# santurini/vsrlab

Hardware: AMD Instinct MI355X
Metric: LR frames/sec fwd+bwd, BasicVSR 4x 540p 7-frame clip, 1->8 MI355X (higher is better)
Workload: dtype bf16; 1 GPU; BasicVSR(mid=64,res_blocks=30,x4) fwd+Charbonnier+bwd+clip+Adam, 540x960->2160x3840, 7-frame clip, 2 clips per GPU (BASELINE configs[1]); clips_per_gpu=2, frames=7, res_blocks=30, parallelism=single GPU, arena=full, train_flow=False, trunk_chains=True

## Files before the change

### __graft_entry__.py

```python
import os
import subprocess
import sys

ROOT = os.path.dirname(os.path.abspath(__file__))
if ROOT not in sys.path:
    sys.path.insert(0, ROOT)


def build() -> None:
    env = dict(os.environ)
    env.setdefault("HIPCC", "/opt/rocm/bin/hipcc" if os.path.exists("/opt/rocm/bin/hipcc") else "hipcc")
    subprocess.run(["make", "-C", os.path.join(ROOT, "vsrlab_amd", "csrc"), "-j4"], check=True, env=env)
    try:
        import json
        head = subprocess.run(["git", "-C", ROOT, "rev-parse", "--short=12", "HEAD"], capture_output=True, text=True).stdout.strip()
        dirty = bool(subprocess.run(["git", "-C", ROOT, "status", "--porcelain", "--", "vsrlab_amd/csrc", "include"],
                                    capture_output=True, text=True).stdout.strip())
        if head:
            with open(os.path.join(ROOT, "vsrlab_amd", "lib", "BUILD_INFO.json"), "w") as f:
                json.dump({"git_head": head, "git_dirty_csrc": dirty}, f)
    except Exception:
        pass
    import vsrlab_amd
    lib = vsrlab_amd._lib.load()
    assert lib.vsr_abi_version() == 4
    vsrlab_amd._lib.load_spatial_corr()
    vsrlab_amd._lib.load_jpeg()
    vsrlab_amd._lib.load_warp_taps()


def smoke() -> None:
    import torch
    from oracle import basicvsr_oracle as O
    from vsrlab_amd.vsr.models.RealBasicVSR.modules.basicvsr import BasicVSR
    assert torch.cuda.is_available(), "smoke() needs an MI355X"
    dev = torch.device("cuda:0")
    shape = (1, 3, 3, 32, 32)
    sd = O.keyed_state_dict(O.basicvsr_param_shapes(64, 2, 4))
    g = torch.Generator().manual_seed(0)
    lrs = torch.rand(*shape, generator=g)
    hr = torch.rand(1, 3, 3, 128, 128, generator=g)
    cot = torch.rand(1, 3, 3, 128, 128, generator=g) * 2 - 1
    sr_o, _, grads_o = O.fwd_bwd({k: v.double() for k, v in sd.items()}, lrs.double(), hr.double(), cot=cot.double())
    _, _, g32 = O.fwd_bwd(sd, lrs, hr, cot=cot)
    with O.emulate_bf16():
        sr_e, _, gemu = O.fwd_bwd(sd, lrs, hr, cot=cot)
    keys = sorted(grads_o)
    cat = lambda d: torch.cat([d[k].double().flatten() for k in keys])
    rel = lambda a, b: float((a - b).norm() / b.norm())
    for dtype, g_cpu, floor, t_sr in (("fp32", g32, 2e-4, 1e-3), ("bf16", gemu, 1e-3, None)):
        m = BasicVSR(64, 2, 4, False, False)
        m.load_state_dict(sd, strict=True)
        m = m.to(dev)
        m.compute_dtype = dtype
        sr = m(lrs.to(dev))
        torch.mean(sr * cot.to(dev)).backward()
        torch.cuda.synchronize()
        e_sr = float((sr.detach().cpu().double() - sr_o).abs().max() / sr_o.abs().max())
        grads = {k: p.grad.cpu() for k, p in m.named_parameters() if p.grad is not None}
        assert set(grads) == set(keys)
        e_g, e_cpu = rel(cat(grads), cat(grads_o)), rel(cat(g_cpu), cat(grads_o))
        print(f"smoke[{dtype}]: sr rel err {e_sr:.3e}, gradient rel-L2 {e_g:.3e} (CPU evaluation at this precision: {e_cpu:.3e}) over {len(keys)} tensors")
        if t_sr is None:
            t_sr = 1.5 * max(float((sr_e.double() - sr_o).abs().max() / sr_o.abs().max()), 1e-3)
        assert e_sr < t_sr and e_g <= 1.5 * max(e_cpu, floor), (dtype, e_sr, e_g, e_cpu)
    from vsrlab_amd import functional as VF
    assert VF.chain_timeouts() == 0, "a trunk-chain dependency wait timed out"
    from vsrlab_amd.core.metrics import PSNR, SSIM, MetricCollection
    from vsrlab_amd.core.utils import compute_metric
    same = compute_metric(MetricCollection({"PSNR": PSNR(), "SSIM": SSIM()}), hr.to(dev), hr.to(dev))
    assert same == {"PSNR": 80.0, "SSIM": 1.0}, same
    from vsrlab_amd.vsr.models.VRT.vrt import aligned_input
    clip = lrs.to(dev)
    zero = torch.zeros(1, 2, 2, 32, 32, device=dev)
    al = aligned_input(clip, zero, zero)
    assert al.shape == (1, 3, 27, 32, 32) and torch.equal(al[:, :, :3], clip)
    assert torch.equal(al[:, :2, 3:15], clip[:, 1:].repeat(1, 1, 4, 1, 1)) and not al[:, 2, 3:15].any()
    assert torch.equal(al[:, 1:, 15:], clip[:, :2].repeat(1, 1, 4, 1, 1)) and not al[:, 0, 15:].any()
    print("smoke OK")


if __name__ == "__main__":
    build()
    if len(sys.argv) > 1 and sys.argv[1] == "smoke":
        smoke()
```

### vsrlab_amd/_lib.py

```python
import ctypes
import os
from ctypes import c_char_p, c_float, c_int, c_longlong, c_size_t, c_void_p

_HERE = os.path.dirname(os.path.abspath(__file__))
LIB_PATH = os.environ.get("VSRLAB_AMD_LIB") or os.path.join(_HERE, "lib", "libvsrlab_hip.so")

DT_F32 = 0
DT_BF16 = 1


class BasicVSRDesc(ctypes.Structure):
    _fields_ = [("n", c_int), ("t", c_int), ("h", c_int), ("w", c_int), ("mid_channels", c_int),
                ("res_blocks", c_int), ("upscale", c_int), ("dtype", c_int), ("arena_mode", c_int)]


class DiscDesc(ctypes.Structure):
    _fields_ = [("n", c_int), ("h", c_int), ("w", c_int), ("mid_ch", c_int), ("dtype", c_int)]


class PerceptualDesc(ctypes.Structure):
    _fields_ = [("n", c_int), ("h", c_int), ("w", c_int), ("dtype", c_int), ("need_grad", c_int)]


class AttnDesc(ctypes.Structure):
    _fields_ = [(k, c_int) for k in ("B", "N", "heads", "head_dim", "q0", "k0", "o0", "Nq", "Nk", "Cout", "c_off", "nW", "Nm")] + \
               [("scale", c_float), ("dtype", c_int), ("mask_packed", c_int), ("mask_value", c_float)]


class DeformDesc(ctypes.Structure):
    _fields_ = [(k, c_int) for k in ("N", "Cin", "Cout", "H", "W", "deform_groups", "modulated", "flow_guided")] + \
               [("max_residue", c_float), ("dtype", c_int)]


class MetricsDesc(ctypes.Structure):
    _fields_ = [("planes", c_longlong), ("C", c_int), ("H", c_int), ("W", c_int), ("window_size", c_int),
                ("sigma", c_float), ("c1", c_float), ("c2", c_float), ("clamp_x", c_int), ("clamp_lo", c_float), ("clamp_hi", c_float)]


class RaftCorrDesc(ctypes.Structure):
    _fields_ = [(k, c_int) for k in ("N", "D", "H", "W", "levels", "radius", "dtype")]


class SpatialCorrDesc(ctypes.Structure):
    _fields_ = [(k, c_int) for k in ("N", "C", "H", "W", "patch_h", "patch_w", "stride_h", "stride_w", "pad_h", "pad_w", "dil_h", "dil_w",
                                     "dtype")] + [("scale", c_float)]


class JpegDesc(ctypes.Structure):
    _fields_ = [(k, c_int) for k in ("N", "H", "W", "quality", "x_dtype", "y_dtype")] + \
               [("x_stride", c_longlong * 4), ("y_stride", c_longlong * 4)]


class WarpTapsDesc(ctypes.Structure):
    _fields_ = [(k, c_int) for k in ("N", "D", "C", "H", "W", "taps", "border", "dtype")] + [("x_nstride", c_longlong)]


_P = c_void_p
_SIGNATURES = {
    "vsr_abi_version": (c_int, []),
    "vsr_status_string": (c_char_p, [c_int]),
    "vsr_basicvsr_num_params": (c_int, [ctypes.POINTER(BasicVSRDesc)]),
    "vsr_basicvsr_workspace_bytes": (c_size_t, [ctypes.POINTER(BasicVSRDesc), c_int]),
    "vsr_basicvsr_forward": (c_int, [ctypes.POINTER(BasicVSRDesc), _P, c_int, _P, _P, _P, c_size_t, c_int, _P]),
    "vsr_basicvsr_backward": (c_int, [ctypes.POINTER(BasicVSRDesc), _P, _P, c_int, _P, _P, _P, _P, c_size_t, _P]),
    "vsr_basicvsr_get_flows": (c_int, [ctypes.POINTER(BasicVSRDesc), _P, _P, _P, _P]),
    "vsr_basicvsr_narrow_workspace_bytes": (c_size_t, [ctypes.POINTER(BasicVSRDesc), c_int]),
    "vsr_basicvsr_narrow_forward": (c_int, [ctypes.POINTER(BasicVSRDesc), _P, c_int, _P, _P, _P, c_size_t, c_int, _P]),
    "vsr_basicvsr_narrow_backward": (c_int, [ctypes.POINTER(BasicVSRDesc), _P, _P, c_int, _P, _P, _P, _P, c_size_t, _P]),
    "vsr_basicvsr_narrow_get_flows": (c_int, [ctypes.POINTER(BasicVSRDesc), _P, _P, _P, _P]),
    "vsr_spynet_workspace_bytes": (c_size_t, [c_int, c_int, c_int, c_int, c_int]),
    "vsr_spynet_forward": (c_int, [c_int, c_int, c_int, c_int, _P, c_int, _P, _P, _P, _P, c_size_t, c_int, _P]),
    "vsr_spynet_backward": (c_int, [c_int, c_int, c_int, c_int, _P, c_int, _P, _P, c_size_t, _P]),
    "vsr_spynet_forward_ex": (c_int, [c_int, c_int, c_int, c_int, _P, c_int, _P, _P, c_int, _P, _P, c_size_t, c_int, _P]),
    "vsr_spynet_backward_ex": (c_int, [c_int, c_int, c_int, c_int, _P, _P, c_int, _P, c_int, _P, _P, _P, _P, c_size_t, _P]),
    "vsr_cleaner_workspace_bytes": (c_size_t, [c_int, c_int, c_int, c_int, c_int, c_int, c_int]),
    "vsr_cleaner_narrow_workspace_bytes": (c_size_t, [c_int, c_int, c_int, c_int, c_int, c_int, c_int, c_int]),
    "vsr_cleaner_forward": (c_int, [c_int, c_int, c_int, c_int, c_int, c_int, c_int, _P, c_int, _P, _P, _P, c_size_t, c_int, _P]),
    "vsr_cleaner_backward": (c_int, [c_int, c_int, c_int, c_int, c_int, c_int, c_int, _P, c_int, _P, _P, _P, _P, c_size_t, _P]),
    "vsr_flow_warp_fwd": (c_int, [c_int, _P, _P, _P, c_int, c_int, c_int, c_int, _P]),
    "vsr_flow_warp_bwd": (c_int, [c_int, _P, _P, _P, c_int, c_int, c_int, c_int, _P]),
    "vsr_flow_warp_bwd_flow": (c_int, [c_int, _P, _P, _P, _P, c_int, c_int, c_int, c_int, _P]),
    "vsr_flow_warp_fwd_ex": (c_int, [c_int, _P, _P, _P, c_int, c_int, c_int, c_int, c_int, _P]),
    "vsr_flow_warp_bwd_ex": (c_int, [c_int, _P, _P, _P, c_int, c_int, c_int, c_int, c_int, _P]),
    "vsr_flow_warp_bwd_flow_ex": (c_int, [c_int, _P, _P, _P, _P, c_int, c_int, c_int, c_int, c_int, _P]),
    "vsr_planar_to_pm": (c_int, [c_int, _P, _P, c_int, c_int, c_int, c_int, c_int, _P]),
    "vsr_pm_to_planar": (c_int, [c_int, _P, _P, c_int, c_int, c_int, c_int, c_int, _P]),
    "vsr_conv3x3_c64_fwd": (c_int, [c_int, _P, _P, _P, _P, _P, _P, c_int, c_int, c_int, c_int, _P]),
    "vsr_conv3x3_c64_chain_sync_bytes": (c_size_t, [c_int, c_int, c_int, c_int]),
    "vsr_conv3x3_c64_chain_fwd": (c_int, [_P, _P, _P, c_int, c_int, c_int, c_int, _P, _P]),
    "vsr_conv3x3_c64_dgrad": (c_int, [c_int, _P, _P, _P, _P, _P, _P, c_int, c_int, c_int, c_int, _P]),
    "vsr_conv_layer_fwd": (c_int, [c_int, c_int, _P, c_int, _P, _P, _P, c_int, c_int, _P, _P, c_int, _P, c_int, c_float, c_int, c_int, c_int, c_int, _P]),
    "vsr_conv_layer_bwd_scratch_bytes": (c_size_t, [c_int, c_int, c_int, c_int, c_int]),
    "vsr_conv_layer_bwd": (c_int, [c_int, c_int, _P, c_int, _P, _P, c_int, c_int, _P, _P, _P, _P, c_int, c_int, c_float, c_int, _P, _P, _P, _P,
                                   _P, c_size_t, c_int, c_int, c_int, _P]),
    "vsr_conv3x3_c64_wgrad_slab_floats": (c_size_t, []),
    "vsr_conv3x3_c64_wgrad": (c_int, [c_int, _P, _P, _P, _P, _P, c_int, c_int, c_int, _P]),
    "vsr_charbonnier_scratch_floats": (c_size_t, []),
    "vsr_charbonnier_fwd_bwd": (c_int, [_P, _P, _P, _P, _P, c_longlong, c_float, _P]),
    "vsr_optim_scratch_floats": (c_size_t, []),
    "vsr_adam_clip_step": (c_int, [_P, _P, _P, _P, c_longlong, c_float, c_float, c_float, c_float, c_float, c_int, c_float,
                                   c_float, _P, _P, _P]),
    "vsr_grad_norm": (c_int, [_P, c_longlong, c_float, _P, _P, _P]),
    "vsr_resize_bilinear": (c_int, [_P, _P, c_longlong, c_int, c_int, c_int, c_int, _P]),
    "vsr_disc_workspace_bytes": (c_size_t, [ctypes.POINTER(DiscDesc), c_int]),
    "vsr_disc_forward": (c_int, [ctypes.POINTER(DiscDesc), _P, c_int, _P, _P, _P, c_size_t, c_int, _P]),
    "vsr_disc_backward": (c_int, [ctypes.POINTER(DiscDesc), _P, c_int, _P, _P, _P, _P, c_size_t, _P]),
    "vsr_spectral_norm": (c_int, [_P, _P, _P, _P, _P, c_int, c_int, c_int, _P]),
    "vsr_spectral_norm_backward": (c_int, [_P, _P, _P, _P, _P, _P, c_int, c_int, _P, _P]),
    "vsr_bce_with_logits": (c_int, [_P, c_float, _P, _P, c_longlong, _P]),
    "vsr_perceptual_workspace_bytes": (c_size_t, [ctypes.POINTER(PerceptualDesc)]),
    "vsr_perceptual_loss": (c_int, [ctypes.POINTER(PerceptualDesc), _P, c_int, _P, _P, _P, _P, _P, _P, c_size_t, _P]),
    "vsr_window_attention_fwd": (c_int, [ctypes.POINTER(AttnDesc), _P, _P, _P, _P, _P, _P]),
    "vsr_window_attention_bwd": (c_int, [ctypes.POINTER(AttnDesc), _P, _P, _P, _P, _P, _P, _P, _P, _P]),
    "vsr_mask_pack": (c_int, [_P, _P, c_int, c_int, _P]),
    "vsr_rpb_gather": (c_int, [_P, _P, c_int, _P, c_int, c_int, _P]),
    "vsr_rpb_scatter": (c_int, [_P, _P, c_int, _P, c_int, c_int, _P]),
    "vsr_deform_conv_workspace_bytes": (c_size_t, [ctypes.POINTER(DeformDesc), c_int]),
    "vsr_deform_conv_fwd": (c_int, [ctypes.POINTER(DeformDesc), _P, _P, _P, _P, _P, _P, _P, _P, c_size_t, _P]),
    "vsr_deform_conv_bwd": (c_int, [ctypes.POINTER(DeformDesc), _P, _P, _P, _P, _P, _P, _P, _P, _P, _P, _P, _P, _P, c_size_t, _P]),
    "vsr_deform_offset_mask": (c_int, [ctypes.POINTER(DeformDesc), _P, _P, _P, _P, _P]),
    "vsr_metrics_scratch_bytes": (c_size_t, [ctypes.POINTER(MetricsDesc)]),
    "vsr_psnr_ssim": (c_int, [ctypes.POINTER(MetricsDesc), _P, _P, _P, _P, c_size_t, _P]),
    "vsr_raft_corr_workspace_bytes": (c_size_t, [ctypes.POINTER(RaftCorrDesc), c_int]),
    "vsr_raft_corr_pyramid_fwd": (c_int, [ctypes.POINTER(RaftCorrDesc), _P, _P, _P, c_size_t, _P]),
    "vsr_raft_corr_pyramid_bwd": (c_int, [ctypes.POINTER(RaftCorrDesc), _P, c_size_t, _P, _P, _P]),
    "vsr_raft_corr_lookup_fwd": (c_int, [ctypes.POINTER(RaftCorrDesc), _P, c_size_t, _P, _P, _P]),
    "vsr_raft_corr_lookup_bwd": (c_int, [ctypes.POINTER(RaftCorrDesc), _P, c_size_t, _P, _P, _P, c_size_t, _P]),
}
EXPORTS = tuple(_SIGNATURES)

OTHER_DEBUG_EXPORTS = ("vsr_debug_chain_inject_error", "vsr_debug_chain_item", "vsr_debug_chain_timeouts", "vsr_debug_chain_timing_begin",
                       "vsr_debug_chain_timing_read", "vsr_debug_warp_bwd_gather", "vsr_debug_warp_bwd_gather_c")
_LL = c_longlong
DEBUG_SIGNATURES = {
    "vsr_debug_tail_last2_fwd": (c_int, [c_int, _P, _P, _P, _P, _P, _P, _LL, _P, _P, _LL, c_int, c_int, c_int, c_int, c_int, c_int, c_int, _P]),
    "vsr_debug_tail_last2_dgrad": (c_int, [_P, _LL, _P, _P, c_int, _P, c_int, c_float, _P, c_int, c_int, c_int, _P]),
    "vsr_debug_tail_planar_c64": (c_int, [c_int, _P, _LL, c_int, _P, _P, _P, _P, c_int, c_float, _P, c_int, c_int, c_int, c_int, _P]),
    "vsr_debug_tail_last2_wgrad": (c_int, [c_int, _P, _P, _LL, c_int, _P, _P, _P, c_int, c_int, c_int, _P]),
    "vsr_debug_tail_conv_unshuffle": (c_int, [c_int, _P, _P, _P, c_int, _P, _P, c_int, c_int, c_int, _P]),
    "vsr_debug_tail_ps_dgrad": (c_int, [c_int, _P, _P, _P, _P, _P, c_int, c_int, _P, c_int, c_int, c_int, c_int, c_int, _P]),
    "vsr_debug_tail_ps_wgrads": (c_int, [c_int, _P, _P, c_int, _P, _P, _P, c_int, c_int, c_int, _P]),
    "vsr_debug_trunk_conv": (c_int, [c_int, c_int, c_int, c_int, _P, _P, _P, _P, _P, c_int, c_float, _P, _P, c_int, _P, _P, c_int, c_int,
                                     c_int, c_int, c_int, _P]),
    "vsr_debug_trunk_stem": (c_int, [c_int, c_int, c_int, _P, _P, _LL, _P, _P, _P, _P, c_int, c_float, c_int, c_int, c_int, _P]),
    "vsr_debug_trunk_stem_dgrad": (c_int, [c_int, c_int, c_int, _P, _P, _P, _P, _P, _LL, c_int, c_int, c_int, c_int, _P]),
    "vsr_debug_trunk_point": (c_int, [c_int, c_int, c_int, _P, _P, _P, _P, _P, _P, _P, c_int, c_int, c_int, _P]),
    "vsr_debug_trunk_wgrad_cc": (c_int, [c_int, c_int, c_int, _P, _P, c_int, _P, c_int, c_int, _P, c_int, _P, c_int, c_int, c_int, _P]),
    "vsr_debug_trunk_stem_wgrads": (c_int, [c_int, c_int, c_int, _P, _LL, _P, c_int, _P, _P, c_int, _P, _P, c_int, _P, c_int, c_int, c_int, _P]),
    "vsr_debug_trunk_chain": (c_int, [c_int, c_int, _P, _P, _P, c_int, _P, c_int, c_int, c_int, c_int, _P]),
    "vsr_debug_spy_conv": (c_int, [c_int, c_int, _P, _P, _P, _P, _P, c_int, _P, c_int, c_int, c_int, _P]),
    "vsr_debug_spy_dgrad": (c_int, [c_int, c_int, _P, _P, _P, _P, _P, c_int, c_int, c_int, _P]),
    "vsr_debug_spy_wgrad": (c_int, [c_int, c_int, _P, _P, _P, _P, c_int, _P, c_int, c_int, c_int, _P]),
    "vsr_debug_spy_prepare": (c_int, [c_int, _P, _P, _P, _P, c_int, c_int, c_int, c_int, c_int, c_int, c_int, _P]),
    "vsr_debug_spy_prepare_bwd": (c_int, [c_int, _P, _P, _P, _P, _P, _P, c_int, c_int, c_int, c_int, c_int, c_int, _P]),
    "vsr_debug_spy_dres": (c_int, [c_int, _P, _P, _P, c_int, c_int, c_int, _P]),
    "vsr_debug_spy_planar": (c_int, [c_int, _P, _P, _P, _P, _P, _LL, c_int, c_int, c_int, c_int, _P]),
}

SPATIAL_CORR_LIB_PATH = os.path.join(_HERE, "lib", "libvsrlab_spatial_corr.so")
SPATIAL_CORR_SIGNATURES = {
    "vsr_spatial_corr_workspace_bytes": (c_size_t, [ctypes.POINTER(SpatialCorrDesc)]),
    "vsr_spatial_corr_fwd": (c_int, [ctypes.POINTER(SpatialCorrDesc), _P, _P, _P, _P, c_size_t, _P]),
    "vsr_spatial_corr_bwd": (c_int, [ctypes.POINTER(SpatialCorrDesc), _P, _P, _P, _P, _P, _P, c_size_t, _P]),
}
SPATIAL_CORR_EXPORTS = tuple(SPATIAL_CORR_SIGNATURES)

JPEG_LIB_PATH = os.path.join(_HERE, "lib", "libvsrlab_jpeg.so")
JPEG_SIGNATURES = {
    "vsr_jpeg_workspace_bytes": (c_size_t, [ctypes.POINTER(JpegDesc)]),
    "vsr_jpeg_fwd": (c_int, [ctypes.POINTER(JpegDesc), _P, _P, _P, c_size_t, _P]),
}
JPEG_EXPORTS = tuple(JPEG_SIGNATURES)

WARP_TAPS_LIB_PATH = os.path.join(_HERE, "lib", "libvsrlab_warp_taps.so")
WARP_TAPS_SIGNATURES = {
    "vsr_warp_taps_fwd": (c_int, [ctypes.POINTER(WarpTapsDesc), _P, _P, _P, _P]),
    "vsr_warp_taps_bwd": (c_int, [ctypes.POINTER(WarpTapsDesc), _P, _P, _P, _P, _P]),
    "vsr_warp_taps_clip_fwd": (c_int, [ctypes.POINTER(WarpTapsDesc), _P, _P, _P, _P, _P]),
    "vsr_warp_taps_clip_bwd": (c_int, [ctypes.POINTER(WarpTapsDesc), _P, _P, _P, _P, _P, _P]),
}
WARP_TAPS_EXPORTS = tuple(WARP_TAPS_SIGNATURES)

_lib = None
_spatial_corr_lib = None
_jpeg_lib = None
_warp_taps_lib = None


def load_warp_taps():
    global _warp_taps_lib
    if _warp_taps_lib is None:
        if not os.path.exists(WARP_TAPS_LIB_PATH):
            raise RuntimeError(
                f"vsrlab_amd: HIP library not built ({WARP_TAPS_LIB_PATH} missing). Run "
                "`python -c 'import __graft_entry__ as g; g.build()'` or `make -C vsrlab_amd/csrc`.")
        lib = ctypes.CDLL(WARP_TAPS_LIB_PATH)
        for name, (res, args) in WARP_TAPS_SIGNATURES.items():
            fn = getattr(lib, name)
            fn.restype = res
            fn.argtypes = args
        _warp_taps_lib = lib
    return _warp_taps_lib


def load_jpeg():
    global _jpeg_lib
    if _jpeg_lib is None:
        if not os.path.exists(JPEG_LIB_PATH):
            raise RuntimeError(
                f"vsrlab_amd: HIP library not built ({JPEG_LIB_PATH} missing). Run "
                "`python -c 'import __graft_entry__ as g; g.build()'` or `make -C vsrlab_amd/csrc`.")
        lib = ctypes.CDLL(JPEG_LIB_PATH)
        for name, (res, args) in JPEG_SIGNATURES.items():
            fn = getattr(lib, name)
            fn.restype = res
            fn.argtypes = args
        _jpeg_lib = lib
    return _jpeg_lib


def load_spatial_corr():
    global _spatial_corr_lib
    if _spatial_corr_lib is None:
        if not os.path.exists(SPATIAL_CORR_LIB_PATH):
            raise RuntimeError(
                f"vsrlab_amd: HIP library not built ({SPATIAL_CORR_LIB_PATH} missing). Run "
                "`python -c 'import __graft_entry__ as g; g.build()'` or `make -C vsrlab_amd/csrc`.")
        lib = ctypes.CDLL(SPATIAL_CORR_LIB_PATH)
        for name, (res, args) in SPATIAL_CORR_SIGNATURES.items():
            fn = getattr(lib, name)
            fn.restype = res
            fn.argtypes = args
        _spatial_corr_lib = lib
    return _spatial_corr_lib


def load():
    global _lib
    if _lib is None:
        if not os.path.exists(LIB_PATH):
            raise RuntimeError(
                f"vsrlab_amd: HIP library not built ({LIB_PATH} missing). Run "
                "`python -c 'import __graft_entry__ as g; g.build()'` or `make -C vsrlab_amd/csrc`.")
        lib = ctypes.CDLL(LIB_PATH)
        for name, (res, args) in _SIGNATURES.items():
            fn = getattr(lib, name)
            fn.restype = res
            fn.argtypes = args
        for name, (res, args) in DEBUG_SIGNATURES.items():
            fn = getattr(lib, name, None) if os.environ.get("VSRLAB_AMD_LIB") else getattr(lib, name)
            if fn is not None:
                fn.restype = res
                fn.argtypes = args
        _lib = lib
    return _lib


def check(status, what):
    if status != 0:
        msg = load().vsr_status_string(status).decode()
        raise RuntimeError(f"vsrlab_amd: {what} failed: {msg} (status {status})")
```

### vsrlab_amd/csrc/common.h

```cpp
#pragma once
#include <hip/hip_runtime.h>
#include <stdint.h>

#define VSR_OK 0
#define VSR_ERR_BADARG (-1)
#define VSR_ERR_UNSUPPORTED (-2)
#define VSR_ERR_HIP (-3)
#define VSR_ERR_WORKSPACE (-4)

#define VSR_F32 0
#define VSR_BF16 1

typedef __bf16 bf16_t;
typedef __attribute__((ext_vector_type(8))) __bf16 bf16x8_t;
typedef __attribute__((ext_vector_type(4))) __bf16 bf16x4_t;
typedef __attribute__((ext_vector_type(4))) short s16x4_t;
typedef __attribute__((ext_vector_type(16))) float f32x16_t;
typedef __attribute__((ext_vector_type(4))) float f32x4_t;

#define VSR_MAX_SRC 4
#define VSR_MAX_Z 4

enum { ACT_NONE = 0, ACT_RELU = 1, ACT_LEAKY = 2 };
enum { MASK_NONE = 0, MASK_RELU = 1, MASK_LEAKY = 2, MASK_RELU_BITS = 3, MASK_LEAKY_BITS = 4 };
enum { EPI_NHWC = 0, EPI_PLANAR = 1 };

struct ConvArgs {
    const void* src[VSR_MAX_SRC];
    long long src_nstride[VSR_MAX_SRC];
    int src_oy[VSR_MAX_SRC], src_ox[VSR_MAX_SRC];
    int in_step, Hs, Ws;
    int N, H, W;
    const void* wpack;
    long long w_zstride;
    const float* bias;
    int bias_zstride;
    int nz;
    void* dst[VSR_MAX_Z];
    long long dst_nstride;
    int out_step, Hd, Wd;
    int out_oy[VSR_MAX_Z], out_ox[VSR_MAX_Z];
    int CD;
    int cout_real;
    int act;
    const void* res[VSR_MAX_Z];
    const void* aux[VSR_MAX_Z];
    int mask_mode;
    const float* pres;
    const float* base_lr;
    long long base_nstride;
    int base_h, base_w, base_scale;
    void* sign_out[VSR_MAX_Z];
    const void* sign_bits[VSR_MAX_Z];
    float leaky_slope;
    int planar_c;
    int unshuffle;
    long long unshuffle_plane;
};
static inline __host__ __device__ float vsr_slope(float s) { return s != 0.f ? s : 0.1f; }

#define VSR_WG_MAXSEG 8
struct WgradArgs {
    const void* x[VSR_WG_MAXSEG];
    const void* dy[VSR_WG_MAXSEG];
    long long x_nstride, dy_nstride;
    int nseg;
    int N, H, W;
    int x_step, x_oy, x_ox, Hx, Wx;
    int dy_step, dy_oy, dy_ox, Hy, Wy;
    float* slab;
    int tap_begin;
    int x_ctotal, x_coff;
    int dy_ctotal, dy_coff;
    int dy_planar_c;
    int slab_stride;
    int ntiles_x, ntiles_y;
    int pair_ksplit, pair_nsl, pair_ncob, pair_views;
};

static inline __host__ __device__ int cdiv(int a, int b) { return (a + b - 1) / b; }
static inline int grid_for(long long total, int block = 256) {
    long long g = (total + block - 1) / block;
    return (int)(g < 1 ? 1 : (g > 256 * 16 ? 256 * 16 : g));
}

static inline __host__ __device__ int pm_ws(int W) { return (W + 31) >> 5; }
static inline __host__ __device__ long long pm_image_elems(int H, int W, int C) { return (long long)H * pm_ws(W) * 32 * C; }
static inline __host__ __device__ long long pm_off(int y, int x, int chunk, int W, int C) {
    const int seg = x >> 5;
    return (((long long)y * pm_ws(W) + seg) * (C >> 3) + chunk) * 256 + (x & 31) * 8;
}

static inline __host__ __device__ int pm_acc_chan(int mb, int row) { return 8 * (4 * (mb >> 1) + (row >> 2)) + 4 * (mb & 1) + (row & 3); }
#define PM_LANE_PIXEL(l15) (((l15) >= 4 && (l15) < 12) ? 2 * ((l15) - 4) : ((l15) < 4 ? 2 * (l15) + 1 : 2 * ((l15) - 8) + 1))

struct TileWalk { int first, end, stride; };
static inline __device__ TileWalk xcd_tile_walk(int total, int block, int nblocks) {
    TileWalk w;
    if (nblocks >= 8 && (nblocks & 7) == 0) {
        const int xcd = block & 7, j = block >> 3;
        const int lo = (int)((long long)xcd * total / 8), hi = (int)((long long)(xcd + 1) * total / 8);
        w.first = lo + j; w.end = hi; w.stride = nblocks >> 3;
    } else {
        w.first = block; w.end = total; w.stride = nblocks;
    }
    return w;
}

#define VSR_MAX_DEVICES 32
struct VsrDevOnce { bool done[VSR_MAX_DEVICES] = {}; };
static inline int vsr_set_max_dynamic_lds(VsrDevOnce& once, const void* kernel, int bytes) {
    int dev = 0;
    if (hipGetDevice(&dev) != hipSuccess) return VSR_ERR_HIP;
    if (dev < 0 || dev >= VSR_MAX_DEVICES) return VSR_ERR_UNSUPPORTED;
    if (!__atomic_load_n(&once.done[dev], __ATOMIC_ACQUIRE)) {
        if (hipFuncSetAttribute(kernel, hipFuncAttributeMaxDynamicSharedMemorySize, bytes) != hipSuccess) return VSR_ERR_HIP;
        __atomic_store_n(&once.done[dev], true, __ATOMIC_RELEASE);
    }
    return VSR_OK;
}

static inline int vsr_num_cus() {
    static int cus[VSR_MAX_DEVICES] = {};
    int dev = 0;
    if (hipGetDevice(&dev) != hipSuccess || dev < 0 || dev >= VSR_MAX_DEVICES) return 256;
    int v = __atomic_load_n(&cus[dev], __ATOMIC_RELAXED);
    if (v == 0) {
        hipDeviceProp_t prop;
        v = (hipGetDeviceProperties(&prop, dev) == hipSuccess && prop.multiProcessorCount > 0) ? prop.multiProcessorCount : 256;
        __atomic_store_n(&cus[dev], v, __ATOMIC_RELAXED);
    }
    return v;
}

#include <cstdlib>
struct VsrEnvSwitches {
    bool generic_conv, generic_wgrad, single_stream;
    int wide2_max_wg;
};
static inline const VsrEnvSwitches& vsr_env() {
    static const VsrEnvSwitches s = [] {
        auto on = [](const char* n) { const char* e = getenv(n); return e && e[0] == '1'; };
        VsrEnvSwitches v;
        v.generic_conv = on("VSRLAB_AMD_GENERIC_CONV");
        v.generic_wgrad = on("VSRLAB_AMD_GENERIC_WGRAD");
        v.single_stream = on("VSRLAB_AMD_SINGLE_STREAM");
        const char* e = getenv("VSRLAB_AMD_WIDE2_MAX_WG");
        v.wide2_max_wg = e ? atoi(e) : 0;
        return v;
    }();
    return s;
}

#define HIP_CHECK_RET(expr)                                   \
    do {                                                      \
        hipError_t _e = (expr);                               \
        if (_e != hipSuccess) return VSR_ERR_HIP;             \
    } while (0)
```

### vsrlab_amd/csrc/engine.hip

```cpp
#include <vector>
#include "recipes.h"
#include "spynet_engine.h"

namespace {

struct Plan {
    VsrBasicVSRDesc d = {};
    int C = 64, CO = 64;
    bool sb = false;
    bool bwd = false, flowgrad = false;
    bool diet = false;
    int rb = 0, n = 0, t = 0, h = 0, w = 0, dtype = VSR_F32;
    int scale = 4, ups = 2;
    bool unsh = false;
    size_t es = 4;
    size_t px1 = 0;
    size_t s_elems = 0;
    size_t stem_w[2] = {}, stem_wd[2] = {}, stem_b[2] = {};
    std::vector<size_t> blk_w[2], blk_wd[2], blk_b[2];
    size_t point_w = 0, point_wd = 0, point_b = 0;
    size_t up_w[2] = {}, up_wd[2] = {}, up_b[2] = {};
    size_t last0_w = 0, last0_wd = 0, last0_b = 0, last2_w = 0, last2_wd = 0, last2_b = 0;
    SpyPlan spy;
    size_t flows = 0;
    std::vector<size_t> Wp[2], X[2], A[2];
    std::vector<size_t> SB[2];
    std::vector<size_t> feat[2];
    size_t scratchA[2] = {}, scratchW[2] = {};
    std::vector<size_t> Pt, U0, U1, C0;
    std::vector<size_t> SBC0;
    std::vector<size_t> SBPt;
    std::vector<size_t> SBX0[2];
    std::vector<size_t> G0[2], G1[2], DX[2];
    std::vector<size_t> dFeatB, dFF;
    size_t S[2] = {}, dWp[2] = {}, slab[2] = {};
    size_t far_cnt = 0;
    size_t chain_sync[2] = {0, 0};
    bool chains = true;
    size_t G_C0 = 0, G_U1 = 0, G_U0 = 0, G_P = 0;
    bool hrdef = false;
    std::vector<size_t> GU1f, GU0f, GPf;
    size_t dflows = 0;
    size_t stem_wd_lr[2] = {};
    size_t total = 0;

    size_t xoff(int dir, int i, int b) const { return X[dir][(size_t)i * (rb + 1) + b]; }
    size_t aoff(int dir, int i, int b) const { return A[dir][(size_t)i * rb + b]; }
    size_t sboff(int dir, int i, int b) const { return SB[dir][(size_t)i * rb + b]; }
    size_t g1off(int dir, int i, int b) const { return diet ? G1[dir][b & 1] : G1[dir][(size_t)i * rb + b]; }
    size_t dxoff(int dir, int i, int b) const { return diet ? DX[dir][b & 1] : DX[dir][(size_t)i * (rb + 1) + b]; }

    int build(const VsrBasicVSRDesc& desc, int mode, bool narrow = false) {
        d = desc; bwd = mode >= 1; flowgrad = mode >= 2;
        { const char* e = getenv("VSRLAB_AMD_CHAIN"); chains = !(e && e[0] == '0'); }
        if (d.arena_mode != 0 && d.arena_mode != 1) return VSR_ERR_BADARG;
        diet = bwd && d.arena_mode == 1;
        rb = d.res_blocks; n = d.n; t = d.t; h = d.h; w = d.w; dtype = d.dtype;
        scale = d.upscale; ups = scale / 2; unsh = false;
        const bool width_ok = narrow ? (d.mid_channels == 16 || d.mid_channels == 32) : d.mid_channels == 64;
        if (!width_ok || (scale != 4 && scale != 2) || rb < 1 || n < 1 || t < 1 || t > 32 || h < 1 || w < 1) return VSR_ERR_UNSUPPORTED;
        if (dtype != VSR_F32 && dtype != VSR_BF16) return VSR_ERR_BADARG;
        const int C = d.mid_channels;
        this->C = C; CO = C < 32 ? 32 : C;
        sb = bwd && dtype == VSR_BF16 && C == 64;
        es = esize(dtype);
        px1 = (size_t)n * pm_image_elems(h, w, C);
        s_elems = (size_t)n * h * w * C;
        const size_t a2 = (size_t)n * pm_image_elems(2 * h, 2 * w, C) * es, a4 = (size_t)n * pm_image_elems(scale * h, scale * w, C) * es;
        const size_t a4h = (size_t)n * pm_image_elems(scale * h, scale * w, 64) * es;
        Bump b;
        const size_t w64 = (size_t)9 * CO * C * es;
        for (int dir = 0; dir < 2; ++dir) {
            stem_w[dir] = b.take(w64 + (size_t)9 * CO * 16 * es);
            stem_wd[dir] = b.take(w64);
            stem_b[dir] = b.take(C * 4);
            blk_w[dir].resize(2 * rb); blk_wd[dir].resize(2 * rb); blk_b[dir].resize(2 * rb);
            for (int k = 0; k < 2 * rb; ++k) { blk_w[dir][k] = b.take(w64); blk_wd[dir][k] = b.take(w64); blk_b[dir][k] = b.take(C * 4); }
        }
        point_w = b.take((size_t)2 * CO * C * es); point_wd = b.take((size_t)2 * CO * C * es); point_b = b.take(C * 4);
        for (int k = 0; k < 2; ++k) { up_w[k] = b.take(4 * w64); up_wd[k] = b.take(4 * w64); up_b[k] = b.take(4 * C * 4); }
        last0_w = b.take((size_t)9 * 64 * C * es); last0_wd = b.take((size_t)9 * CO * 64 * es); last0_b = b.take(64 * 4);
        last2_w = b.take((size_t)9 * 32 * 64 * es); last2_wd = b.take((size_t)9 * 64 * 16 * es); last2_b = b.take(64 * 4);
        if (t > 1) spy.plan(b, 2 * n * (t - 1), n * t, h, w, dtype);
        flows = b.take((size_t)2 * n * (t > 1 ? t - 1 : 1) * 2 * h * w * 4);
        const size_t a1 = px1 * es;
        for (int dir = 0; dir < 2; ++dir) {
            Wp[dir].assign(t, 0); feat[dir].assign(t, 0);
            if (bwd) {
                X[dir].assign((size_t)t * (rb + 1), 0); A[dir].assign((size_t)t * rb, 0); SB[dir].assign((size_t)t * rb, 0);
                SBX0[dir].assign(t, 0);
                const size_t sbytes = sb ? (size_t)n * cdiv(h, 8) * cdiv(w, 32) * 2048 : 256;
                for (int i = 0; i < t; ++i) {
                    SBX0[dir][i] = b.take(sbytes);
                    Wp[dir][i] = b.take(a1);
                    for (int k = 0; k <= rb; ++k) X[dir][(size_t)i * (rb + 1) + k] = b.take(a1);
                    for (int k = 0; k < rb; ++k) A[dir][(size_t)i * rb + k] = b.take(a1);
                    for (int k = 0; k < rb; ++k) SB[dir][(size_t)i * rb + k] = b.take(sbytes);
                    feat[dir][i] = xoff(dir, i, rb);
                }
            } else {
                for (int i = 0; i < t; ++i) feat[dir][i] = b.take(a1);
            }
        }
        for (int dir = 0; dir < 2; ++dir) { scratchA[dir] = b.take(a1); scratchW[dir] = b.take(a1); }
        const int nrec = bwd ? t : 1;
        Pt.assign(t, 0); U0.assign(t, 0); U1.assign(t, 0); C0.assign(t, 0);
        for (int i = 0; i < nrec; ++i) {
            Pt[i] = b.take(a1);
            if (diet && i > 0) { U0[i] = U0[0]; U1[i] = U1[0]; C0[i] = C0[0]; } else { U0[i] = b.take(a2); U1[i] = ups == 2 ? b.take(a4) : U0[i]; C0[i] = b.take(a4h); }
        }
        for (int i = nrec; i < t; ++i) { Pt[i] = Pt[0]; U0[i] = U0[0]; U1[i] = U1[0]; C0[i] = C0[0]; }
        SBC0.assign(t, 0); SBPt.assign(t, 0);
        if (sb)
            for (int i = 0; i < t; ++i) {
                SBC0[i] = b.take((size_t)n * cdiv(scale * h, 8) * cdiv(scale * w, 32) * 2048);
                SBPt[i] = b.take((size_t)n * cdiv(h, 8) * cdiv(w, 32) * 2048);
            }
        if (bwd) {
            for (int dir = 0; dir < 2; ++dir) {
                G0[dir].assign(t, 0);
                for (int i = 0; i < t; ++i) G0[dir][i] = b.take(a1);
                if (diet) {
                    G1[dir].assign(2, 0); DX[dir].assign(2, 0);
                    for (int k = 0; k < 2; ++k) { G1[dir][k] = b.take(a1); DX[dir][k] = b.take(a1); }
                } else if (dir == 0) {
                    G1[dir].assign((size_t)t * rb, 0); DX[dir].assign((size_t)t * (rb + 1), 0);
                    for (int i = 0; i < t; ++i) {
                        for (int k = 0; k < rb; ++k) G1[dir][(size_t)i * rb + k] = b.take(a1);
                        for (int k = 1; k <= rb; ++k) DX[dir][(size_t)i * (rb + 1) + k] = b.take(a1);
                    }
                } else {
                    G1[dir] = G1[0]; DX[dir] = DX[0];
                }
            }
            dFeatB.assign(t, 0); dFF.assign(t, 0);
            for (int i = 0; i < t; ++i) { dFeatB[i] = b.take(a1); dFF[i] = b.take(a1); }
            for (int dir = 0; dir < 2; ++dir) { S[dir] = b.take(s_elems * 8); dWp[dir] = b.take(a1); }
            far_cnt = b.take((size_t)2 * 32 * 4);
            G_C0 = b.take(a4h); G_P = b.take(a1);
            unsh = !diet && dtype == VSR_BF16 && !vsr_env().generic_conv && C == 64;
            const size_t gu1 = unsh && 4 * a2 > a4 ? 4 * a2 : a4, gu0 = unsh && 4 * a1 > a2 ? 4 * a1 : a2;
            if (ups == 2) { if (diet) { G_U1 = C0[0]; G_U0 = U1[0]; } else { G_U1 = b.take(gu1); G_U0 = b.take(gu0); } }
            else { G_U0 = diet ? C0[0] : b.take(gu0); G_U1 = G_U0; }
            hrdef = unsh;
            GU1f.assign(t, G_U1); GU0f.assign(t, G_U0); GPf.assign(t, G_P);
            if (hrdef)
                for (int i = 1; i < t; ++i) {
                    GU0f[i] = b.take(gu0);
                    GU1f[i] = ups == 2 ? b.take(gu1) : GU0f[i];
                    GPf[i] = b.take(a1);
                }
            for (int k = 0; k < 2; ++k) slab[k] = b.take(wgrad_slab_bytes());
        }
        for (int dir = 0; dir < 2; ++dir) chain_sync[dir] = sb ? b.take(vsr_chain_sync_bytes(VSR_CHAIN_MAX_LAYERS, n, h, w)) : 0;
        dflows = 0;
        if (flowgrad && t > 1) {
            dflows = b.take((size_t)2 * n * (t - 1) * 2 * h * w * 4);
            spy.plan_save(b, dtype);
        }
        if (flowgrad) {
            for (int dir = 0; dir < 2; ++dir) stem_wd_lr[dir] = b.take((size_t)9 * 32 * C * es);
        }
        total = b.off;
        return VSR_OK;
    }
};

Ctx engine_ctx(const Plan& p, char* ws, hipStream_t st, int lane) {
    return Ctx(ws, st, p.dtype, p.C, p.bwd ? reinterpret_cast<float*>(ws + p.slab[lane]) : nullptr);
}

struct PIdx {
    int rb;
    int ups = 2;
    int trunk_base(int dir) const { return dir * (2 + 4 * rb); }
    int stem_w(int dir) const { return trunk_base(dir); }
    int stem_b(int dir) const { return trunk_base(dir) + 1; }
    int blk_w(int dir, int k) const { return trunk_base(dir) + 2 + 2 * k; }
    int blk_b(int dir, int k) const { return trunk_base(dir) + 3 + 2 * k; }
    int point_w() const { return 2 * (2 + 4 * rb); }
    int point_b() const { return point_w() + 1; }
    int up_w(int k) const { return point_w() + 2 + 2 * k; }
    int up_b(int k) const { return up_w(k) + 1; }
    int last0_w() const { return point_w() + 2 + 2 * ups; }
    int last0_b() const { return last0_w() + 1; }
    int last2_w() const { return last0_w() + 2; }
    int last2_b() const { return last0_w() + 3; }
    int spy_base() const { return last0_w() + 4; }
    int spy_w(int lvl, int j) const { return spy_base() + (lvl * NSPY + j) * 2; }
    int spy_b(int lvl, int j) const { return spy_w(lvl, j) + 1; }
    int spy_mean() const { return spy_base() + 60; }
    int spy_std() const { return spy_base() + 61; }
    int count() const { return spy_base() + 62; }
};

int pack_all_collect(const Ctx& c, const Plan& p, const float* const* prm);
int pack_all(const Ctx& c, const Plan& p, const float* const* prm) {
    std::vector<VsrPackDesc> descs;
    descs.reserve(512);
    c.batch = &descs;
    const int rc = pack_all_collect(c, p, prm);
    c.batch = nullptr;
    if (rc != VSR_OK) return rc;
    return vsr_launch_pack_multi(descs.data(), (int)descs.size(), c.st);
}

int pack_all_collect(const Ctx& c, const Plan& p, const float* const* prm) {
    const PIdx ix{p.rb, p.ups};
    const int C = p.C, CO = p.CO;
    for (int dir = 0; dir < 2; ++dir) {
        const float* sw = prm[ix.stem_w(dir)];
        CK(c.pack_stem(sw, c.at(p.stem_w[dir]), true));
        CK(c.pack_bias(prm[ix.stem_b(dir)], c.at(p.stem_b[dir]), C));
        if (p.bwd) CK(c.pack_stem_dgrad(sw, c.at(p.stem_wd[dir])));
        if (p.flowgrad) CK(c.pack_stem_dlr(sw, c.at(p.stem_wd_lr[dir]), true));
        for (int k = 0; k < 2 * p.rb; ++k) {
            CK(c.pack_cc(3, prm[ix.blk_w(dir, k)], c.at(p.blk_w[dir][k]), 0));
            if (p.bwd) CK(c.pack_cc(3, prm[ix.blk_w(dir, k)], c.at(p.blk_wd[dir][k]), 1));
            CK(c.pack_bias(prm[ix.blk_b(dir, k)], c.at(p.blk_b[dir][k]), C));
        }
    }
    CK(c.pack_point(prm[ix.point_w()], c.at(p.point_w), 0));
    if (p.bwd) CK(c.pack_point(prm[ix.point_w()], c.at(p.point_wd), 1));
    CK(c.pack_bias(prm[ix.point_b()], c.at(p.point_b), C));
    for (int k = 0; k < p.ups; ++k) {
        CK(c.pack_ps(prm[ix.up_w(k)], c.at(p.up_w[k]), 0));
        if (p.bwd) CK(c.pack_ps(prm[ix.up_w(k)], c.at(p.up_wd[k]), 1));
        CK(c.pack_ps_bias(prm[ix.up_b(k)], (float*)c.at(p.up_b[k])));
    }
    CK(c.pack(prm[ix.last0_w()], c.at(p.last0_w), 9, 64, C, 64, C, C, 0, 1, 0, 0));
    if (p.bwd) CK(c.pack(prm[ix.last0_w()], c.at(p.last0_wd), 9, CO, 64, C, 64, C, 0, 1, 0, 1));
    CK(c.pack_bias(prm[ix.last0_b()], c.at(p.last0_b), 64));
    CK(c.pack(prm[ix.last2_w()], c.at(p.last2_w), 9, 32, 64, 3, 64, 64, 0, 1, 0, 0));
    if (p.bwd) CK(c.pack(prm[ix.last2_w()], c.at(p.last2_wd), 9, 64, 16, 64, 3, 64, 0, 1, 0, 1));
    CK(c.pack_bias(prm[ix.last2_b()], c.at(p.last2_b), 3));
    if (p.t > 1) CK(vsr::spynet_pack(c, p.spy, prm, ix.spy_base()));
    return VSR_OK;
}

bool chain_on(const Plan& p) { return p.chains && p.chain_sync[0] && p.chain_sync[1] && 2 * p.rb <= VSR_CHAIN_MAX_LAYERS; }
unsigned chain_off(size_t o) { return (unsigned)(o >> 8); }
int chain_launch(const ChainArgs& a, hipStream_t st) {
    const size_t img_bytes = (size_t)pm_image_elems(a.H, a.W, 64) * 2, sb_bytes = (size_t)cdiv(a.H, 8) * cdiv(a.W, 32) * 2048;
    if (a.N > 1 && img_bytes * 3 * a.N > ((size_t)192 << 20) && cdiv(a.H, 8) * cdiv(a.W, 32) >= 2 * vsr_num_cus()) {
        for (int m = 0; m < a.N; ++m) {
            ChainArgs b = a;
            b.N = 1;
            const unsigned di = (unsigned)((m * img_bytes) >> 8), ds = (unsigned)((m * sb_bytes) >> 8);
            for (int l = 0; l < a.nlayers; ++l) {
                ChainLayer& L = b.layer[l];
                L.src += di; L.dst += di;
                if (L.res != 0xffffffffu) L.res += di;
                if (L.sbits != 0xffffffffu) L.sbits += ds;
                if (L.sout != 0xffffffffu) L.sout += ds;
            }
            CK(chain_launch(b, st));
        }
        return VSR_OK;
    }
    return vsr_launch_conv3x3_chain(a, vsr_num_cus(), st);
}
int trunk_chain_forward(const Ctx& c, const Plan& p, int dir, int i) {
    ChainArgs a = {};
    a.base = c.ws; a.sync = (unsigned*)c.at(p.chain_sync[dir]); a.N = p.n; a.H = p.h; a.W = p.w; a.nlayers = 2 * p.rb;
    for (int b = 0; b < p.rb; ++b) {
        ChainLayer& l1 = a.layer[2 * b];
        l1 = {chain_off(p.xoff(dir, i, b)), chain_off(p.aoff(dir, i, b)), 0xffffffffu, 0xffffffffu, chain_off(p.sboff(dir, i, b)),
              chain_off(p.blk_w[dir][2 * b]), chain_off(p.blk_b[dir][2 * b]), CHAIN_RELU};
        ChainLayer& l2 = a.layer[2 * b + 1];
        l2 = {chain_off(p.aoff(dir, i, b)), chain_off(p.xoff(dir, i, b + 1)), chain_off(p.xoff(dir, i, b)), 0xffffffffu, 0xffffffffu,
              chain_off(p.blk_w[dir][2 * b + 1]), chain_off(p.blk_b[dir][2 * b + 1]), CHAIN_SKIP};
    }
    return chain_launch(a, c.st);
}
int trunk_chain_backward(const Ctx& c, const Plan& p, int dir, int i) {
    ChainArgs a = {};
    a.base = c.ws; a.sync = (unsigned*)c.at(p.chain_sync[dir]); a.N = p.n; a.H = p.h; a.W = p.w;
    int L = 0;
    for (int b = p.rb - 1; b >= 0; --b) {
        a.layer[L++] = {chain_off(p.dxoff(dir, i, b + 1)), chain_off(p.g1off(dir, i, b)), 0xffffffffu, chain_off(p.sboff(dir, i, b)), 0xffffffffu,
                        chain_off(p.blk_wd[dir][2 * b + 1]), 0xffffffffu, CHAIN_MASK};
        if (b > 0)
            a.layer[L++] = {chain_off(p.g1off(dir, i, b)), chain_off(p.dxoff(dir, i, b)), chain_off(p.dxoff(dir, i, b + 1)), 0xffffffffu, 0xffffffffu,
                            chain_off(p.blk_wd[dir][2 * b]), 0xffffffffu, CHAIN_SKIP};
    }
    a.nlayers = L;
    return chain_launch(a, c.st);
}

int trunk_forward(const Ctx& c, const Plan& p, int dir, int i, const void* warped, const float* lrs) {
    const int n = p.n, h = p.h, w = p.w, rb = p.rb;
    void* x = p.bwd ? c.at(p.xoff(dir, i, 0)) : c.at(p.feat[dir][i]);
    {
        CK(c.stem(true, warped, lrs + (size_t)i * 3 * h * w, (long long)p.t * 3 * h * w, c.at(p.stem_w[dir]), c.fat(p.stem_b[dir]), x, ACT_LEAKY, 0.f, n, h, w));
        if (p.sb) CK(vsr_launch_sign_bits_c64(x, c.at(p.SBX0[dir][i]), n, h, w, c.st));
    }
    if (chain_on(p)) return trunk_chain_forward(c, p, dir, i);
    for (int b = 0; b < rb; ++b) {
        void* act = p.bwd ? c.at(p.aoff(dir, i, b)) : c.at(p.scratchA[dir]);
        void* xn = p.bwd ? c.at(p.xoff(dir, i, b + 1)) : x;
        CK(c.conv(3, x, c.at(p.blk_w[dir][2 * b]), c.fat(p.blk_b[dir][2 * b]), act, ACT_RELU, nullptr, nullptr, 0, n, h, w,
                    p.sb ? c.at(p.sboff(dir, i, b)) : nullptr));
        CK(c.conv(3, act, c.at(p.blk_w[dir][2 * b + 1]), c.fat(p.blk_b[dir][2 * b + 1]), xn, ACT_NONE, x, nullptr, 0, n, h, w));
        x = xn;
    }
    return VSR_OK;
}

int last0_forward(const Ctx& c, const Plan& p, int i, void* sign_out) {
    const int S = p.scale;
    if (p.C == 64)
        return c.conv(3, c.at(p.U1[i]), c.at(p.last0_w), c.fat(p.last0_b), c.at(p.C0[i]), ACT_LEAKY, nullptr, nullptr, 0, p.n, S * p.h, S * p.w, sign_out);
    ConvArgs a = conv_args(p.n, S * p.h, S * p.w, c.C);
    a.src[0] = c.at(p.U1[i]); a.wpack = c.at(p.last0_w); a.bias = c.fat(p.last0_b); a.dst[0] = c.at(p.C0[i]); a.act = ACT_LEAKY;
    a.CD = 64; a.cout_real = 64; a.dst_nstride = pm_image_elems(S * p.h, S * p.w, 64);
    return vsr_launch_conv(c.dtype, 3, 1, p.C, p.C, 0, 64, EPI_NHWC, a, c.st);
}

int recon_forward(const Ctx& c, const Plan& p, int i, const float* lrs, float* sr) {
    const int n = p.n, h = p.h, w = p.w;
    CK(c.point_conv(c.at(p.feat[0][i]), c.at(p.feat[1][i]), c.at(p.point_w), c.fat(p.point_b), c.at(p.Pt[i]), n, h, w));
    if (p.sb) CK(vsr_launch_sign_bits_c64(c.at(p.Pt[i]), c.at(p.SBPt[i]), n, h, w, c.st));
    const int S = p.scale;
    CK(c.conv_ps(c.at(p.Pt[i]), c.at(p.up_w[0]), c.fat(p.up_b[0]), c.at(p.U0[i]), n, h, w));
    if (p.ups == 2) CK(c.conv_ps(c.at(p.U0[i]), c.at(p.up_w[1]), c.fat(p.up_b[1]), c.at(p.U1[i]), n, 2 * h, 2 * w));
    CK(last0_forward(c, p, i, p.sb ? c.at(p.SBC0[i]) : nullptr));
    {
        ConvArgs a = conv_args(n, S * h, S * w, c.C);
        a.src_nstride[0] = pm_image_elems(S * h, S * w, 64);
        a.src[0] = c.at(p.C0[i]); a.wpack = c.at(p.last2_w); a.bias = c.fat(p.last2_b); a.cout_real = 3;
        a.dst[0] = sr + (size_t)i * 3 * S * S * h * w; a.dst_nstride = (long long)p.t * 3 * S * S * h * w;
        a.base_lr = lrs + (size_t)i * 3 * h * w; a.base_nstride = (long long)p.t * 3 * h * w; a.base_h = h; a.base_w = w; a.base_scale = S;
        CK(vsr_launch_conv(c.dtype, 3, 1, 64, 64, 0, 32, EPI_PLANAR, a, c.st));
    }
    return VSR_OK;
}

const float* flow_ptr(const Ctx& c, const Plan& p, int forward, int i) {
    return c.fat(p.flows) + ((size_t)forward * p.n * (p.t - 1) + i) * 2 * p.h * p.w;
}

struct Helper { hipStream_t s = nullptr; hipEvent_t fork = nullptr, join = nullptr; int dev = -1; };
int get_helper(Helper** out) {
    thread_local Helper hp[16];
    int dev = 0;
    HIP_CHECK_RET(hipGetDevice(&dev));
    if (dev < 0 || dev >= 16) return VSR_ERR_UNSUPPORTED;
    Helper& x = hp[dev];
    if (!x.s) {
        HIP_CHECK_RET(hipStreamCreateWithFlags(&x.s, hipStreamNonBlocking));
        HIP_CHECK_RET(hipEventCreateWithFlags(&x.fork, hipEventDisableTiming));
        HIP_CHECK_RET(hipEventCreateWithFlags(&x.join, hipEventDisableTiming));
        x.dev = dev;
    }
    *out = &x;
    return VSR_OK;
}
bool single_stream() { return vsr_env().single_stream; }
struct Fork {
    hipStream_t main; Helper* h; bool active = false;
    int begin(bool fork = true) {
        if (single_stream() || !fork) return VSR_OK;
        CK(get_helper(&h));
        HIP_CHECK_RET(hipEventRecord(h->fork, main));
        HIP_CHECK_RET(hipStreamWaitEvent(h->s, h->fork, 0));
        active = true;
        return VSR_OK;
    }
    hipStream_t side() const { return active ? h->s : main; }
    int end() {
        if (!active) return VSR_OK;
        active = false;
        HIP_CHECK_RET(hipEventRecord(h->join, h->s));
        HIP_CHECK_RET(hipStreamWaitEvent(main, h->join, 0));
        return VSR_OK;
    }
    ~Fork() { (void)end(); }
};

int forward_chain(const Ctx& c, const Plan& p, int dir, const float* lrs) {
    const int n = p.n, t = p.t, h = p.h, w = p.w;
    const long long fstride = (long long)(t - 1) * 2 * h * w;
    for (int k = 0; k < t; ++k) {
        const int i = dir == 0 ? t - 1 - k : k;
        void* warped = nullptr;
        if (k > 0) {
            const int prev = dir == 0 ? i + 1 : i - 1;
            warped = p.bwd ? c.at(p.Wp[dir][i]) : c.at(p.scratchW[dir]);
            CK(vsr_launch_warp_fwd(c.dtype, c.at(p.feat[dir][prev]), flow_ptr(c, p, dir, dir == 0 ? i : i - 1), warped, n, h, w, p.C, fstride, c.st));
        }
        CK(trunk_forward(c, p, dir, i, warped, lrs));
    }
    return VSR_OK;
}

int forward_impl(const Plan& p, const float* const* prm, const float* lrs, float* sr, char* ws, hipStream_t st) {
    const Ctx c = engine_ctx(p, ws, st, 0);
    const PIdx ix{p.rb, p.ups};
    const int n = p.n, t = p.t;
    CK(pack_all(c, p, prm));
    if (t > 1) CK(vsr::spynet_run(c, p.spy, lrs, prm[ix.spy_mean()], prm[ix.spy_std()], n, t, 0, (float*)c.at(p.flows)));
    {
        Fork f{st, nullptr};
        CK(f.begin(!chain_on(p)));
        const Ctx c0 = engine_ctx(p, ws, st, 0), c1 = engine_ctx(p, ws, f.side(), 1);
        CK(forward_chain(c0, p, 0, lrs));
        CK(forward_chain(c1, p, 1, lrs));
        CK(f.end());
    }
    for (int i = 0; i < t; ++i) CK(recon_forward(c, p, i, lrs, sr));
    return VSR_OK;
}

int recon_ps_wgrads(const Ctx& c, const Plan& p, int k, int f0, int f1, float* const* g) {
    const PIdx ix{p.rb, p.ups};
    const int H = (k + 1) * p.h, W = (k + 1) * p.w;
    for (int i0 = f0; i0 < f1; i0 += VSR_WG_MAXSEG) {
        const int i1 = i0 + VSR_WG_MAXSEG < f1 ? i0 + VSR_WG_MAXSEG : f1;
        const void* x[VSR_WG_MAXSEG];
        const void* dy[VSR_WG_MAXSEG];
        for (int i = i0; i < i1; ++i) { x[i - i0] = c.at(k == 1 ? p.U0[i] : p.Pt[i]); dy[i - i0] = c.at(k == 1 ? p.GU1f[i] : p.GU0f[i]); }
        CK(c.ps_wgrads(x, dy, i1 - i0, p.unsh, p.n, H, W, g[ix.up_w(k)], g[ix.up_b(k)], 1));
    }
    return VSR_OK;
}
int recon_point_wgrads(const Ctx& c, const Plan& p, int f0, int f1, float* const* g) {
    const PIdx ix{p.rb, p.ups};
    const int C = p.C;
    for (int i0 = f0; i0 < f1; i0 += VSR_WG_MAXSEG) {
        const int i1 = i0 + VSR_WG_MAXSEG < f1 ? i0 + VSR_WG_MAXSEG : f1;
        for (int s = 0; s < 2; ++s) {
            WgradArgs a = wg_base(p.n, p.h, p.w, C, C);
            a.nseg = 0;
            for (int i = i0; i < i1; ++i) { a.x[a.nseg] = c.at(p.feat[s][i]); a.dy[a.nseg] = c.at(p.GPf[i]); ++a.nseg; }
            CK(c.wgrad_cc(1, a, g[ix.point_w()], 2 * C, s * C, s == 0 ? g[ix.point_b()] : nullptr, 1));
        }
    }
    return VSR_OK;
}

int recon_backward(const Ctx& c, const Plan& p, int i, const float* lrs, const float* dsr, float* const* g, const float* last2_w) {
    const PIdx ix{p.rb, p.ups};
    if (p.diet) {
        CK(c.conv_ps(c.at(p.Pt[i]), c.at(p.up_w[0]), c.fat(p.up_b[0]), c.at(p.U0[i]), p.n, p.h, p.w));
        if (p.ups == 2) CK(c.conv_ps(c.at(p.U0[i]), c.at(p.up_w[1]), c.fat(p.up_b[1]), c.at(p.U1[i]), p.n, 2 * p.h, 2 * p.w));
        CK(last0_forward(c, p, i, nullptr));
    }
    const int C = p.C;
    const int n = p.n, h = p.h, w = p.w, H4 = p.scale * h, W4 = p.scale * w;
    const float* dsr_i = dsr + (size_t)i * 3 * H4 * W4;
    const long long dsr_ns = (long long)p.t * 3 * H4 * W4;
    if (c.dtype == VSR_BF16 && last2_w) {
        CK(vsr_launch_last2_dgrad(dsr_i, dsr_ns, last2_w, c.at(p.C0[i]), c.at(p.G_C0), n, H4, W4, MASK_LEAKY, c.st, p.sb ? c.at(p.SBC0[i]) : nullptr));
    } else {
        ConvArgs a = conv_args(n, H4, W4, c.C);
        a.src[0] = dsr_i; a.src_nstride[0] = dsr_ns; a.wpack = c.at(p.last2_wd); a.dst[0] = c.at(p.G_C0);
        a.aux[0] = c.at(p.C0[i]); a.mask_mode = MASK_LEAKY;
        a.CD = 64; a.cout_real = 64; a.dst_nstride = pm_image_elems(H4, W4, 64);
        CK(vsr_launch_conv(c.dtype, 3, 1, 16, 16, 1, 64, EPI_NHWC, a, c.st));
    }
    {
        WgradArgs a = wg_base(n, H4, W4, 64, 64);
        a.x[0] = c.at(p.C0[i]); a.dy[0] = dsr_i; a.dy_nstride = dsr_ns;
        CK(c.wgrad(a, {3, 64, false, 16, true}, {3, 64, g[ix.last2_w()], 64, 0, 1, 0, g[ix.last2_b()], 1}));
    }
    const size_t gu1 = p.GU1f[i], gu0 = p.GU0f[i], gp = p.GPf[i];
    if (C == 64) {
        CK(c.conv(3, c.at(p.G_C0), c.at(p.last0_wd), nullptr, c.at(gu1), ACT_NONE, nullptr, nullptr, 0, n, H4, W4, nullptr, nullptr, p.unsh));
    } else {
        ConvArgs a = conv_args(n, H4, W4, c.C);
        a.src[0] = c.at(p.G_C0); a.src_nstride[0] = pm_image_elems(H4, W4, 64); a.wpack = c.at(p.last0_wd); a.dst[0] = c.at(gu1);
        CK(vsr_launch_conv(c.dtype, 3, 1, 64, 64, 0, p.CO, EPI_NHWC, a, c.st));
    }
    {
        WgradArgs a = wg_base(n, H4, W4, C, 64);
        a.x[0] = c.at(p.U1[i]); a.dy[0] = c.at(p.G_C0);
        CK(c.wgrad(a, {3, C, false, 64, false}, {64, C, g[ix.last0_w()], C, 0, 1, 0, g[ix.last0_b()], 1}));
    }
    if (p.ups == 2) {
        CK(c.conv_ps_dgrad(c.at(gu1), c.at(p.up_wd[1]), c.at(gu0), nullptr, 0, n, 2 * h, 2 * w, nullptr, p.unsh, p.unsh));
        if (!p.hrdef) CK(recon_ps_wgrads(c, p, 1, i, i + 1, g));
    }
    CK(c.conv_ps_dgrad(c.at(gu0), c.at(p.up_wd[0]), c.at(gp), c.at(p.Pt[i]), MASK_LEAKY, n, h, w, p.sb ? c.at(p.SBPt[i]) : nullptr, p.unsh, false));
    if (!p.hrdef) CK(recon_ps_wgrads(c, p, 0, i, i + 1, g));
    CK(c.point_dgrad(c.at(gp), c.at(p.point_wd), c.at(p.dFeatB[i]), c.at(p.dFF[i]), n, h, w));
    if (!p.hrdef) CK(recon_point_wgrads(c, p, i, i + 1, g));
    return VSR_OK;
}

int stem_wgrads(const Ctx& c, const Plan& p, int dir, int f0, int f1, const float* lrs, float* const* g);
int block_wgrads(const Ctx& c, const Plan& p, int dir, int b, int f0, int f1, float* const* g);
int trunk_backward(const Ctx& c, const Plan& p, int dir, int i, const void* dtop, const float* pending_flow, int pending_k, bool has_warp,
                   const float* lrs, float* const* g) {
    const int n = p.n, h = p.h, w = p.w, rb = p.rb;
    if (pending_flow) {
        const long long fstride = (long long)(p.t - 1) * 2 * h * w;
        CK(vsr_launch_warp_bwd_gather(c.dtype, c.at(p.dWp[dir]), pending_flow, dtop, (long long*)c.at(p.S[dir]),
                                      (int*)c.at(p.far_cnt) + dir * 32 + pending_k, c.at(p.dxoff(dir, i, rb)), n, h, w, p.C, fstride, c.st));
    } else {
        CK(vsr_launch_add_cast(c.dtype, dtop, nullptr, c.at(p.dxoff(dir, i, rb)), n, h, w, p.C, c.st));
    }
    const bool chain = chain_on(p) && !p.diet;
    if (chain) CK(trunk_chain_backward(c, p, dir, i));
    for (int b = chain ? 0 : rb - 1; b >= 0; --b) {
        const void* dxn = c.at(p.dxoff(dir, i, b + 1));
        if (!chain) CK(c.conv(3, dxn, c.at(p.blk_wd[dir][2 * b + 1]), nullptr, c.at(p.g1off(dir, i, b)), ACT_NONE, nullptr, c.at(p.aoff(dir, i, b)), MASK_RELU, n, h, w,
                    nullptr, p.sb ? c.at(p.sboff(dir, i, b)) : nullptr));
        void* out = b > 0 ? c.at(p.dxoff(dir, i, b)) : c.at(p.G0[dir][i]);
        CK(c.conv(3, c.at(p.g1off(dir, i, b)), c.at(p.blk_wd[dir][2 * b]), nullptr, out, ACT_NONE, dxn, b == 0 ? c.at(p.xoff(dir, i, 0)) : nullptr,
                    b == 0 ? MASK_LEAKY : 0, n, h, w, nullptr, (b == 0 && p.sb) ? c.at(p.SBX0[dir][i]) : nullptr));
        if (p.diet) CK(block_wgrads(c, p, dir, b, i, i + 1, g));
    }
    if (has_warp)
        CK(c.conv(3, c.at(p.G0[dir][i]), c.at(p.stem_wd[dir]), nullptr, c.at(p.dWp[dir]), ACT_NONE, nullptr, nullptr, 0, n, h, w));
    if (p.diet) CK(stem_wgrads(c, p, dir, i, i + 1, lrs, g));
    return VSR_OK;
}

int stem_wgrads(const Ctx& c, const Plan& p, int dir, int f0, int f1, const float* lrs, float* const* g) {
    const PIdx ix{p.rb, p.ups};
    const int n = p.n, t = p.t, h = p.h, w = p.w, C = p.C;
    WgradArgs a = wg_base(n, h, w, C, C), af = a;
    a.nseg = af.nseg = 0;
    a.x_nstride = (long long)t * 3 * h * w;
    for (int i = f0; i < f1; ++i) {
        a.x[a.nseg] = lrs + (size_t)i * 3 * h * w; a.dy[a.nseg] = c.at(p.G0[dir][i]); ++a.nseg;
        const bool has = dir == 0 ? (i < t - 1) : (i > 0);
        if (has) { af.x[af.nseg] = c.at(p.Wp[dir][i]); af.dy[af.nseg] = c.at(p.G0[dir][i]); ++af.nseg; }
    }
    return c.stem_wgrads(true, a, af, g[ix.stem_w(dir)], g[ix.stem_b(dir)], 1);
}
int block_wgrads(const Ctx& c, const Plan& p, int dir, int b, int f0, int f1, float* const* g) {
    const PIdx ix{p.rb, p.ups};
    const int C = p.C;
    WgradArgs a1 = wg_base(p.n, p.h, p.w, C, C), a2 = wg_base(p.n, p.h, p.w, C, C);
    a1.nseg = a2.nseg = 0;
    for (int i = f0; i < f1; ++i) {
        a1.x[a1.nseg] = c.at(p.xoff(dir, i, b)); a1.dy[a1.nseg] = c.at(p.g1off(dir, i, b)); ++a1.nseg;
        a2.x[a2.nseg] = c.at(p.aoff(dir, i, b)); a2.dy[a2.nseg] = c.at(p.dxoff(dir, i, b + 1)); ++a2.nseg;
    }
    CK(c.wgrad_cc(3, a1, g[ix.blk_w(dir, 2 * b)], C, 0, g[ix.blk_b(dir, 2 * b)], 1));
    CK(c.wgrad_cc(3, a2, g[ix.blk_w(dir, 2 * b + 1)], C, 0, g[ix.blk_b(dir, 2 * b + 1)], 1));
    return VSR_OK;
}
int trunk_wgrads(const Ctx& c, const Plan& p, int dir, const float* lrs, float* const* g) {
    for (int i0 = 0; i0 < p.t; i0 += VSR_WG_MAXSEG) {
        const int i1 = i0 + VSR_WG_MAXSEG < p.t ? i0 + VSR_WG_MAXSEG : p.t;
        CK(stem_wgrads(c, p, dir, i0, i1, lrs, g));
        for (int b = 0; b < p.rb; ++b) CK(block_wgrads(c, p, dir, b, i0, i1, g));
    }
    return VSR_OK;
}

int backward_chain(const Ctx& c, const Plan& p, int dir, const float* lrs, float* const* g) {
    const int n = p.n, t = p.t, h = p.h, w = p.w;
    const long long fstride = (long long)(t - 1) * 2 * h * w;
    HIP_CHECK_RET(hipMemsetAsync(c.at(p.S[dir]), 0, p.s_elems * 8, c.st));
    HIP_CHECK_RET(hipMemsetAsync((int*)c.at(p.far_cnt) + dir * 32, 0, 32 * 4, c.st));
    const float* pending = nullptr;
    for (int k = 0; k < t; ++k) {
        const int i = dir == 1 ? t - 1 - k : k;
        const void* dtop = dir == 1 ? c.at(p.dFF[i]) : c.at(p.dFeatB[i]);
        const bool last = k == t - 1;
        CK(trunk_backward(c, p, dir, i, dtop, pending, k, !last, lrs, g));
        pending = nullptr;
        if (!last) {
            pending = flow_ptr(c, p, dir, dir == 1 ? i - 1 : i);
            if (p.flowgrad) {
                const int prev = dir == 1 ? i - 1 : i + 1, fi = dir == 1 ? i - 1 : i;
                float* df = (float*)c.at(p.dflows) + ((size_t)dir * p.n * (p.t - 1) + fi) * 2 * p.h * p.w;
                CK(vsr_launch_warp_bwd_flow(c.dtype, c.at(p.feat[dir][prev]), c.at(p.dWp[dir]), flow_ptr(c, p, dir, fi), df, n, h, w, p.C, fstride, c.st));
            }
        }
    }
    return p.diet ? VSR_OK : trunk_wgrads(c, p, dir, lrs, g);
}

int backward_impl(const Plan& p, const float* const* prm, float* const* g, const float* lrs, const float* dsr, float* dlrs,
                  char* ws, hipStream_t st) {
    const Ctx c = engine_ctx(p, ws, st, 0);
    if (dlrs) CK(vsr_launch_bilinear4_bwd(dsr, dlrs, (long long)p.n * p.t * 3, p.h, p.w, st, p.scale));
    for (int i = p.t - 1; i >= 0; --i) CK(recon_backward(c, p, i, lrs, dsr, g, prm ? prm[PIdx{p.rb, p.ups}.last2_w()] : nullptr));
    if (p.hrdef) {
        if (p.ups == 2) CK(recon_ps_wgrads(c, p, 1, 0, p.t, g));
        CK(recon_ps_wgrads(c, p, 0, 0, p.t, g));
        CK(recon_point_wgrads(c, p, 0, p.t, g));
    }
    Fork f{st, nullptr};
    CK(f.begin(p.diet));
    const Ctx c0 = engine_ctx(p, ws, st, 0), c1 = engine_ctx(p, ws, f.side(), 1);
    CK(backward_chain(c0, p, 1, lrs, g));
    CK(backward_chain(c1, p, 0, lrs, g));
    CK(f.end());
    if (dlrs) {
        for (int dir = 0; dir < 2; ++dir)
            for (int i = 0; i < p.t; ++i) {
                float* d = dlrs + (size_t)i * 3 * p.h * p.w;
                CK(c.conv_planar3(c.at(p.G0[dir][i]), c.at(p.stem_wd_lr[dir]), nullptr, d, (long long)p.t * 3 * p.h * p.w, d, p.n, p.h, p.w));
            }
    }
    if (p.flowgrad && p.t > 1)
        CK(vsr::spynet_backward(c, p.spy, c.fat(p.dflows), p.n, p.t, 0, g, PIdx{p.rb, p.ups}.spy_base(), dlrs, prm[PIdx{p.rb, p.ups}.spy_std()]));
    return VSR_OK;
}

}

extern "C" {

int vsr_abi_version(void) { return 4; }

const char* vsr_status_string(int s) {
    switch (s) {
        case VSR_OK: return "ok";
        case VSR_ERR_BADARG: return "bad argument";
        case VSR_ERR_UNSUPPORTED: return "unsupported shape/configuration for the HIP path";
        case VSR_ERR_HIP: return "HIP runtime error";
        case VSR_ERR_WORKSPACE: return "workspace too small";
        default: return "unknown status";
    }
}

int vsr_basicvsr_num_params(const VsrBasicVSRDesc* d) {
    if (!d || d->res_blocks < 0) return VSR_ERR_BADARG;
    return PIdx{d->res_blocks, d->upscale == 2 ? 1 : 2}.count();
}

}

namespace {
size_t basicvsr_workspace_bytes(const VsrBasicVSRDesc* d, int need_backward, bool narrow) {
    if (!d) return 0;
    Plan p;
    if (p.build(*d, need_backward, narrow) != VSR_OK) return 0;
    return p.total;
}

int basicvsr_forward(const VsrBasicVSRDesc* d, const float* const* params, int nparams, const float* lrs, float* sr,
                     void* workspace, size_t workspace_bytes, int need_backward, void* stream, bool narrow) {
    if (!d || !params || !lrs || !sr || !workspace) return VSR_ERR_BADARG;
    Plan p;
    CK(p.build(*d, need_backward, narrow));
    if (nparams != PIdx{p.rb, p.ups}.count()) return VSR_ERR_BADARG;
    for (int k = 0; k < nparams; ++k) if (!params[k]) return VSR_ERR_BADARG;
    if (workspace_bytes < p.total) return VSR_ERR_WORKSPACE;
    return forward_impl(p, params, lrs, sr, (char*)workspace, (hipStream_t)stream);
}

int basicvsr_backward(const VsrBasicVSRDesc* d, const float* const* params, float* const* grads, int nparams,
                      const float* lrs, const float* dsr, float* dlrs, void* workspace, size_t workspace_bytes, void* stream, bool narrow) {
    if (!d || !params || !grads || !lrs || !dsr || !workspace) return VSR_ERR_BADARG;
    if (d->res_blocks < 1) return VSR_ERR_UNSUPPORTED;
    const PIdx ix{d->res_blocks, d->upscale == 2 ? 1 : 2};
    if (nparams != ix.count()) return VSR_ERR_BADARG;
    bool flow = dlrs != nullptr;
    for (int k = ix.spy_base(); k < ix.spy_mean(); ++k) flow = flow || grads[k];
    Plan p;
    CK(p.build(*d, flow ? 2 : 1, narrow));
    if (workspace_bytes < p.total) return VSR_ERR_WORKSPACE;
    return backward_impl(p, params, grads, lrs, dsr, dlrs, (char*)workspace, (hipStream_t)stream);
}

int basicvsr_get_flows(const VsrBasicVSRDesc* d, const void* workspace, float* flow_forward, float* flow_backward, void* stream, bool narrow) {
    if (!d || !workspace) return VSR_ERR_BADARG;
    Plan p;
    CK(p.build(*d, 0, narrow));
    if (p.t < 2) return VSR_OK;
    const size_t half = (size_t)p.n * (p.t - 1) * 2 * p.h * p.w * 4;
    const char* f = (const char*)workspace + p.flows;
    if (flow_backward) HIP_CHECK_RET(hipMemcpyAsync(flow_backward, f, half, hipMemcpyDeviceToDevice, (hipStream_t)stream));
    if (flow_forward) HIP_CHECK_RET(hipMemcpyAsync(flow_forward, f + half, half, hipMemcpyDeviceToDevice, (hipStream_t)stream));
    return VSR_OK;
}
}

extern "C" {
size_t vsr_basicvsr_workspace_bytes(const VsrBasicVSRDesc* d, int need_backward) { return basicvsr_workspace_bytes(d, need_backward, false); }
int vsr_basicvsr_forward(const VsrBasicVSRDesc* d, const float* const* params, int nparams, const float* lrs, float* sr,
                         void* workspace, size_t workspace_bytes, int need_backward, void* stream) {
    return basicvsr_forward(d, params, nparams, lrs, sr, workspace, workspace_bytes, need_backward, stream, false);
}
int vsr_basicvsr_backward(const VsrBasicVSRDesc* d, const float* const* params, float* const* grads, int nparams,
                          const float* lrs, const float* dsr, float* dlrs, void* workspace, size_t workspace_bytes, void* stream) {
    return basicvsr_backward(d, params, grads, nparams, lrs, dsr, dlrs, workspace, workspace_bytes, stream, false);
}
int vsr_basicvsr_get_flows(const VsrBasicVSRDesc* d, const void* workspace, float* flow_forward, float* flow_backward, void* stream) {
    return basicvsr_get_flows(d, workspace, flow_forward, flow_backward, stream, false);
}
size_t vsr_basicvsr_narrow_workspace_bytes(const VsrBasicVSRDesc* d, int need_backward) { return basicvsr_workspace_bytes(d, need_backward, true); }
int vsr_basicvsr_narrow_forward(const VsrBasicVSRDesc* d, const float* const* params, int nparams, const float* lrs, float* sr,
                                void* workspace, size_t workspace_bytes, int need_backward, void* stream) {
    return basicvsr_forward(d, params, nparams, lrs, sr, workspace, workspace_bytes, need_backward, stream, true);
}
int vsr_basicvsr_narrow_backward(const VsrBasicVSRDesc* d, const float* const* params, float* const* grads, int nparams,
                                 const float* lrs, const float* dsr, float* dlrs, void* workspace, size_t workspace_bytes, void* stream) {
    return basicvsr_backward(d, params, grads, nparams, lrs, dsr, dlrs, workspace, workspace_bytes, stream, true);
}
int vsr_basicvsr_narrow_get_flows(const VsrBasicVSRDesc* d, const void* workspace, float* flow_forward, float* flow_backward, void* stream) {
    return basicvsr_get_flows(d, workspace, flow_forward, flow_backward, stream, true);
}

}
```

### vsrlab_amd/csrc/host.h

```cpp
#pragma once
#include "kernels.h"
#include "../../include/vsrlab_hip.h"

#define CK(expr) do { int _s = (expr); if (_s != VSR_OK) return _s; } while (0)

struct Bump {
    size_t off = 0;
    size_t take(size_t bytes) {
        size_t o = off;
        off += (bytes + 255) & ~size_t(255);
        return o;
    }
};

inline size_t esize(int dtype) { return dtype == VSR_BF16 ? 2 : 4; }
inline bool bad_dtype(int dtype) { return dtype != VSR_F32 && dtype != VSR_BF16; }
inline bool bad_dims(int N, int H, int W) { return N < 1 || H < 1 || W < 1; }

inline ConvArgs conv_args(int N, int H, int W, int C) {
    ConvArgs a = {};
    a.in_step = 1; a.Hs = H; a.Ws = W; a.N = N; a.H = H; a.W = W; a.nz = 1;
    a.out_step = 1; a.Hd = H; a.Wd = W; a.CD = C; a.cout_real = C; a.dst_nstride = pm_image_elems(H, W, C);
    for (int s = 0; s < VSR_MAX_SRC; ++s) a.src_nstride[s] = pm_image_elems(H, W, C);
    return a;
}

inline WgradArgs wg_base(int N, int H, int W, int Cx = 64, int Cy = 64) {
    WgradArgs a = {};
    a.N = N; a.H = H; a.W = W; a.nseg = 1;
    a.x_step = 1; a.Hx = H; a.Wx = W; a.x_nstride = pm_image_elems(H, W, Cx);
    a.dy_step = 1; a.Hy = H; a.Wy = W; a.dy_nstride = pm_image_elems(H, W, Cy);
    return a;
}

inline int wgrad_slab_stride3() { int cp, xp, stride; vsr_wgrad_slab_dims(3, 64, 64, &cp, &xp, &stride); return stride; }
inline size_t wgrad_slab_floats() { return (size_t)VSR_WGRAD_NWG * wgrad_slab_stride3(); }
inline size_t wgrad_slab_bytes() { return wgrad_slab_floats() * 4; }

struct WgradShape { int ks, cx; bool x_planar; int cout; bool dy_planar; };
struct WgradDst {
    int cout_real, cin_real; float* gw; int I_total, i_off, o_mul, o_add; float* gb; int accumulate;
};

inline int wgrad_launch(hipStream_t st, int dtype, float* slab, WgradArgs& a, const WgradShape& s, bool even, int* nslabs) {
    int cp, xpd, stride;
    vsr_wgrad_slab_dims(s.ks, s.cx, s.cout, &cp, &xpd, &stride);
    a.slab = slab; a.slab_stride = stride;
    const int tiles = a.N * cdiv(a.H, 8) * cdiv(a.W, 32);
    const long long cap = (long long)wgrad_slab_floats() / stride;
    int nwg = tiles < VSR_WGRAD_NWG ? tiles : VSR_WGRAD_NWG;
    if (nwg > cap) nwg = (int)cap;
    if (even && nwg > 1) nwg &= ~1;
    if (dtype == VSR_BF16 && s.ks == 3 && s.cx == 64 && !s.x_planar && s.cout == 16 && s.dy_planar && a.nseg == 1 && a.x_step == 1 &&
        a.dy_step == 1 && a.Hx == a.H && a.Wx == a.W && a.Hy == a.H && a.Wy == a.W)
        return vsr_launch_last2_wgrad(a.x[0], reinterpret_cast<const float*>(a.dy[0]), a.dy_nstride, slab, stride, a.N, a.H, a.W, nslabs, st,
                                      a.dy_planar_c ? a.dy_planar_c : 3);
    return vsr_launch_wgrad(dtype, s.ks, s.cx, s.x_planar, s.cout, s.dy_planar, a, nwg, nslabs, st);
}
inline int wgrad_run(hipStream_t st, int dtype, float* slab, WgradArgs& a, const WgradShape& s, const WgradDst& d, bool even = true) {
    if (!d.gw && !d.gb) return VSR_OK;
    int nslabs = 0;
    CK(wgrad_launch(st, dtype, slab, a, s, even, &nslabs));
    if (!d.gw) return VSR_ERR_BADARG;
    return vsr_launch_wgrad_reduce(slab, nslabs, s.ks, s.cx, s.cout, d.cout_real, d.cin_real, d.gw, d.I_total, d.i_off, d.o_mul, d.o_add, d.gb,
                                   d.accumulate, st);
}
```

### vsrlab_amd/csrc/kernels.h

```cpp
#pragma once
#include "common.h"

int vsr_launch_conv(int dtype, int ks, int nsrc, int ca, int cb, int last_planar, int cout_t, int epi,
                    const ConvArgs& a, hipStream_t st);
int vsr_launch_sign_bits_c64(const void* x_pm, void* bits, int N, int H, int W, hipStream_t st);

enum { CHAIN_RELU = 0,
       CHAIN_SKIP = 1,
       CHAIN_MASK = 2 };
#define VSR_CHAIN_MAX_LAYERS 64
struct ChainLayer { unsigned src, dst, res, sbits, sout, w, bias; int variant; };
struct ChainArgs {
    char* base;
    unsigned* sync;
    int N, H, W, nlayers;
    ChainLayer layer[VSR_CHAIN_MAX_LAYERS];
};
size_t vsr_chain_sync_bytes(int nlayers, int N, int H, int W);
int vsr_launch_conv3x3_chain(const ChainArgs& a, int num_cus, hipStream_t st);
void vsr_wgrad_slab_dims(int ks, int cx, int cout, int* coutp, int* cxp, int* stride);
int vsr_launch_wgrad(int dtype, int ks, int cx, int x_planar, int cout, int dy_planar, const WgradArgs& a, int nwg,
                     int* nslabs, hipStream_t st);
int vsr_launch_wgrad_reduce(const float* slab, int nwg, int ks, int cx, int cout, int cout_real, int cin_real, float* gw,
                            int I_total, int i_off, int o_mul, int o_add, float* gb, int accumulate, hipStream_t st);
int vsr_launch_warp_fwd(int dtype, const void* in, const float* flow, void* out, int N, int H, int W, int C,
                        long long flow_nstride, hipStream_t st, int border = 0);
int vsr_launch_warp_bwd(int dtype, const void* dout, const float* flow, float* dacc, int N, int H, int W, int C,
                        long long flow_nstride, hipStream_t st, int border = 0);
int vsr_launch_warp_bwd_gather(int dtype, const void* dout, const float* flow, const void* dtop, long long* S, int* far_count, void* out,
                               int N, int H, int W, int C, long long flow_nstride, hipStream_t st);
int vsr_launch_add_cast(int dtype, const void* a, const float* s, void* out, int N, int H, int W, int C, hipStream_t st);
int vsr_launch_planar_to_pm(int dtype, const float* in, void* out, int N, int Cin, int H, int W, int C, hipStream_t st);
int vsr_launch_pm_to_planar(int dtype, const void* in, float* out, int N, int Cout, int H, int W, int C, hipStream_t st);
int vsr_launch_resize_norm(const float* in, float* out, const float* mean, const float* std, int F, int h, int w, int hu,
                           int wu, hipStream_t st);
int vsr_launch_avgpool2(const float* in, float* out, long long planes, int h, int w, hipStream_t st);
int vsr_launch_spynet_prepare(int dtype, const float* frames, const float* flow_prev, float* flow_up, void* x16, int n,
                              int t, int P, int pair_mode, int h, int w, int level0, hipStream_t st);
int vsr_launch_flow_out(const float* in, float* out, int P, int hu, int wu, int h, int w, hipStream_t st);
int vsr_launch_warp_bwd_flow(int dtype, const void* in, const void* dout, const float* flow, float* dflow, int N, int H, int W,
                             int C, long long flow_nstride, hipStream_t st, int border = 0);
int vsr_launch_spynet_dres(int dtype, const float* dflow, const float* res, void* out, int P, int h, int w, hipStream_t st);
int vsr_launch_spynet_prepare_bwd(int dtype, const void* dx16, const float* dflow_l, const float* frames, const float* flow_up,
                                  float* dflow_prev, float* dframes, int n, int t, int P, int pair_mode, int h, int w, hipStream_t st);
int vsr_launch_avgpool2_bwd_add(const float* dcoarse, float* dfine, long long planes, int h, int w, hipStream_t st);
int vsr_launch_resize_norm_bwd(const float* dnorm, float* dframes, const float* std, int F, int h, int w, int hu, int wu, hipStream_t st);
int vsr_launch_bilinear4_bwd(const float* dsr, float* dlr, long long planes, int h, int w, hipStream_t st, int scale = 4);
int vsr_launch_flow_out_bwd(const float* dout, float* din, int P, int hu, int wu, int h, int w, hipStream_t st);
int vsr_launch_add_f32(const float* a, const float* b, float* out, long long n, hipStream_t st);
int vsr_launch_c64_to_planar(const ConvArgs& a, hipStream_t st);
int vsr_launch_last2_wgrad(const void* x, const float* dy, long long dy_nstride, float* slab, int slab_stride, int N, int H, int W,
                           int* nslabs, hipStream_t st, int pc = 3);
int vsr_launch_last2_dgrad(const float* dsr, long long dsr_nstride, const float* w, const void* aux, void* dst, int N, int H, int W,
                           int mask_mode, hipStream_t st, const void* sign_bits = nullptr, float slope = 0.f);
struct VsrPackDesc {
    const float* w; void* dst;
    int total, blk0;
    short KK, RP, CPd, r_real, c_real, I_total, i_off, o_mul, o_add;
    unsigned char mode, dtype;
};
#define VSR_PACK_BATCH 80
int vsr_launch_pack_multi(const VsrPackDesc* descs, int n, hipStream_t st);
int vsr_launch_pack_weights(int dtype, const float* w, void* dst, int KK, int RP, int CPd, int r_real, int c_real,
                            int I_total, int i_off, int o_mul, int o_add, int mode, hipStream_t st);
int vsr_charbonnier_scratch_floats_impl();
int vsr_launch_charbonnier_grad(const float* sr, const float* hr, float* dsr, float* loss_acc, float* scratch, long long n, float eps,
                                hipStream_t st);

struct VsrWideConv {
    const void* x; int xC, Hx, Wx, in_step, nsl;
    int N, H, W;
    const void* wpack; const float* bias;
    void* y; int yC, Hy, Wy, out_step, ncob;
    int act; float slope;
    void* y_act; const void* res; void* y_pre; const void* aux;
    const void* wpack2;
};
int vsr_launch_conv_wide(int dtype, const VsrWideConv& c, hipStream_t st);
long long vsr_wide_pack_elems(int cout, int cin, int mode);
long long vsr_wide2_pack_elems(int cout, int cin, int mode);
int vsr_launch_pack_wide2(const float* w, void* dst, int cout, int cin, int mode, hipStream_t st);
int vsr_launch_pack_wide(int dtype, const float* w, void* dst, int cout, int cin, int mode, hipStream_t st);
int vsr_launch_wgrad_reduce_s2(const float* slab, int nwg, int slab_stride, float* gw, int cin_total, int co0, int ci0, int view, hipStream_t st);
int vsr_launch_up2_fwd(int dtype, const void* a, const void* b, void* out, int N, int H, int W, int C, hipStream_t st);
int vsr_launch_up2_bwd(int dtype, const void* dout, void* din, void* dmask, const void* m, float slope, int N, int H, int W, int C, hipStream_t st);
int vsr_launch_mask_pm(int dtype, const void* g, const void* m, void* out, float slope, long long elems, hipStream_t st);
int vsr_launch_add_pm(int dtype, const void* a, const void* b, void* out, long long elems, hipStream_t st);

#define VSR_WGRAD_MAX_PAIR_SLABS 1024
int vsr_launch_wgrad_pairs(int dtype, const WgradArgs& a, int nsl, int ncob, int views, int ksplit, float* gw, int cin_total, hipStream_t st);
#define VSR_WGRAD_NWG 512
```

### vsrlab_amd/csrc/recipes.h

```cpp
#pragma once
#include <vector>
#include "host.h"

inline constexpr int NSPY = 5;
inline constexpr int SPY_CI[NSPY] = {8, 32, 64, 32, 16};
inline constexpr int SPY_CO[NSPY] = {32, 64, 32, 16, 2};
inline constexpr int SPY_CIP[NSPY] = {16, 32, 64, 32, 16};
inline constexpr int SPY_COP[NSPY] = {32, 64, 32, 32, 32};
inline constexpr int SPY_CD[NSPY] = {32, 64, 32, 16, 0};
inline constexpr int SPY_DK[NSPY] = {32, 64, 32, 16, 16};
inline constexpr int SPY_DROWS[NSPY] = {32, 32, 64, 32, 32};

struct Ctx {
    char* ws;
    hipStream_t st;
    int dtype;
    int C, CO;
    size_t es;
    float* slab;
    mutable std::vector<VsrPackDesc>* batch = nullptr;
    Ctx(char* ws_, hipStream_t st_, int dtype_, int C_ = 64, float* slab_ = nullptr)
        : ws(ws_), st(st_), dtype(dtype_), C(C_), CO(C_ < 32 ? 32 : C_), es(esize(dtype_)), slab(slab_) {}
    void* at(size_t off) const { return ws + off; }
    const float* fat(size_t off) const { return reinterpret_cast<const float*>(ws + off); }

    static long long plane_elems(int N, int H, int W) { return (long long)N * pm_image_elems(H / 2, W / 2, 64); }
    static void set_unshuffle(ConvArgs& a, int N, int H, int W) {
        a.unshuffle = 1; a.unshuffle_plane = plane_elems(N, H, W); a.dst_nstride = pm_image_elems(H / 2, W / 2, 64);
    }
    int conv(int ks, const void* x, const void* wpack, const float* bias, void* y, int act, const void* res, const void* aux, int mask,
             int N, int H, int W, void* sign_out = nullptr, const void* sign_bits = nullptr, bool unshuffle = false, float slope = 0.f) const {
        ConvArgs a = conv_args(N, H, W, C);
        a.src[0] = x; a.wpack = wpack; a.bias = bias; a.dst[0] = y; a.act = act; a.leaky_slope = slope; a.res[0] = res; a.aux[0] = aux; a.mask_mode = mask;
        a.sign_out[0] = sign_out; a.sign_bits[0] = sign_bits;
        if (unshuffle) set_unshuffle(a, N, H, W);
        const int rc = vsr_launch_conv(dtype, ks, 1, C, C, 0, CO, EPI_NHWC, a, st);
        if (rc == VSR_OK && sign_out && dtype == VSR_BF16 && vsr_env().generic_conv) return vsr_launch_sign_bits_c64(y, sign_out, N, H, W, st);
        return rc;
    }
    int conv_planar3(const void* x, const void* wpack, const float* bias, float* y, long long y_nstride, const float* pres, int N, int H, int W) const {
        ConvArgs a = conv_args(N, H, W, C);
        a.src[0] = x; a.wpack = wpack; a.bias = bias; a.cout_real = 3; a.dst[0] = y; a.dst_nstride = y_nstride; a.pres = pres;
        return vsr_launch_conv(dtype, 3, 1, C, C, 0, 32, EPI_PLANAR, a, st);
    }

    int pack_ps(const float* w, void* dst, int mode) const {
        for (int z = 0; z < 4; ++z) CK(pack(w, (char*)dst + (size_t)z * 9 * CO * C * es, 9, CO, C, C, C, C, 0, 4, z, mode));
        return VSR_OK;
    }
    int pack_ps_bias(const float* b, float* dst) const {
        for (int z = 0; z < 4; ++z) CK(pack_bias(b, dst + z * C, C, 4, z));
        return VSR_OK;
    }
    int conv_ps(const void* x, const void* wpack, const float* bias4, void* y, int N, int H, int W, int act = ACT_NONE, float slope = 0.f) const {
        ConvArgs a = conv_args(N, H, W, C);
        a.src[0] = x; a.wpack = wpack; a.w_zstride = 9 * CO * C; a.bias = bias4; a.bias_zstride = C; a.nz = 4; a.act = act; a.leaky_slope = slope;
        a.out_step = 2; a.Hd = 2 * H; a.Wd = 2 * W; a.dst_nstride = pm_image_elems(2 * H, 2 * W, C);
        for (int z = 0; z < 4; ++z) { a.dst[z] = y; a.out_oy[z] = z >> 1; a.out_ox[z] = z & 1; }
        return vsr_launch_conv(dtype, 3, 1, C, C, 0, CO, EPI_NHWC, a, st);
    }
    int conv_ps_dgrad(const void* dy, const void* wpackd, void* dx, const void* aux, int mask, int N, int H, int W, const void* sign_bits = nullptr,
                      bool dy_planes = false, bool dx_planes = false) const {
        if (dtype == VSR_BF16 && C == 64) {
            for (int z = 0; z < 4; ++z) {
                ConvArgs a = conv_args(N, H, W, C);
                if (dy_planes) {
                    a.src[0] = (const char*)dy + (size_t)z * plane_elems(N, 2 * H, 2 * W) * es;
                } else {
                    a.in_step = 2; a.Hs = 2 * H; a.Ws = 2 * W;
                    a.src[0] = dy; a.src_oy[0] = z >> 1; a.src_ox[0] = z & 1; a.src_nstride[0] = pm_image_elems(2 * H, 2 * W, C);
                }
                a.wpack = (const char*)wpackd + (size_t)z * 9 * C * C * es; a.dst[0] = dx;
                a.res[0] = z > 0 ? dx : nullptr;
                if (dx_planes) set_unshuffle(a, N, H, W);
                if (z == 3) { a.aux[0] = aux; a.mask_mode = mask; a.sign_bits[0] = aux ? sign_bits : nullptr; }
                int rc = vsr_launch_conv(dtype, 3, 1, 64, 64, 0, 64, EPI_NHWC, a, st);
                if (rc != VSR_OK) return rc;
            }
            return VSR_OK;
        }
        ConvArgs a = conv_args(N, H, W, C);
        a.nz = 1; a.in_step = 2; a.Hs = 2 * H; a.Ws = 2 * W;
        for (int s = 0; s < 4; ++s) { a.src[s] = dy; a.src_oy[s] = s >> 1; a.src_ox[s] = s & 1; a.src_nstride[s] = pm_image_elems(2 * H, 2 * W, C); }
        a.wpack = wpackd; a.dst[0] = dx; a.aux[0] = aux; a.mask_mode = mask;
        return vsr_launch_conv(dtype, 3, 4, C, C, 0, CO, EPI_NHWC, a, st);
    }
    int ps_wgrads(const void* const* x, const void* const* dy, int nseg, bool dy_planes, int N, int H, int W, float* gw, float* gb, int accumulate) const {
        for (int z = 0; z < 4; ++z) {
            WgradArgs a = wg_base(N, H, W, C, C);
            a.nseg = nseg;
            for (int i = 0; i < nseg; ++i) {
                a.x[i] = x[i];
                a.dy[i] = dy_planes ? (const char*)dy[i] + (size_t)z * plane_elems(N, 2 * H, 2 * W) * es : dy[i];
            }
            if (!dy_planes) { a.dy_step = 2; a.dy_oy = z >> 1; a.dy_ox = z & 1; a.Hy = 2 * H; a.Wy = 2 * W; a.dy_nstride = pm_image_elems(2 * H, 2 * W, C); }
            CK(wgrad(a, {3, C, false, C, false}, {C, C, gw, C, 0, 4, z, gb, accumulate}));
        }
        return VSR_OK;
    }

    int pack_stem(const float* w, void* dst, bool cat) const {
        const int I_total = cat ? C + 3 : 3;
        if (cat) CK(pack(w, dst, 9, CO, C, C, C, I_total, 3, 1, 0, 0));
        return pack(w, (char*)dst + (cat ? (size_t)9 * CO * C * es : 0), 9, CO, 16, C, 3, I_total, 0, 1, 0, 0);
    }
    int pack_stem_dgrad(const float* w, void* dst) const { return pack(w, dst, 9, CO, C, C, C, C + 3, 3, 1, 0, 1); }
    int pack_stem_dlr(const float* w, void* dst, bool cat) const { return pack(w, dst, 9, 32, C, 3, C, cat ? C + 3 : 3, 0, 1, 0, 1); }
    int stem(bool cat, const void* feat, const float* lr, long long lr_nstride, const void* wpack, const float* bias, void* y, int act, float slope,
             int N, int H, int W) const {
        ConvArgs a = conv_args(N, H, W, C);
        a.wpack = wpack; a.bias = bias; a.dst[0] = y; a.act = act; a.leaky_slope = slope;
        a.src[cat ? 1 : 0] = lr; a.src_nstride[cat ? 1 : 0] = lr_nstride;
        if (!cat) return vsr_launch_conv(dtype, 3, 1, 16, 16, 1, CO, EPI_NHWC, a, st);
        a.src[0] = feat;
        return vsr_launch_conv(dtype, 3, 2, C, 16, 1, CO, EPI_NHWC, a, st);
    }
    int stem_wgrads(bool cat, WgradArgs& a_lr, WgradArgs& a_feat, float* gw, float* gb, int accumulate) const {
        const int I_total = cat ? C + 3 : 3;
        CK(wgrad(a_lr, {3, 16, true, C, false}, {C, 3, gw, I_total, 0, 1, 0, gb, accumulate}));
        if (cat && a_feat.nseg) CK(wgrad_cc(3, a_feat, gw, I_total, 3, nullptr, accumulate));
        return VSR_OK;
    }

    int pack_point(const float* w, void* dst, int mode) const {
        for (int s = 0; s < 2; ++s) CK(pack(w, (char*)dst + (size_t)s * CO * C * es, 1, CO, C, C, C, 2 * C, s * C, 1, 0, mode));
        return VSR_OK;
    }
    int point_conv(const void* xa, const void* xb, const void* wpack, const float* bias, void* y, int N, int H, int W) const {
        ConvArgs a = conv_args(N, H, W, C);
        a.src[0] = xa; a.src[1] = xb;
        a.wpack = wpack; a.bias = bias; a.dst[0] = y; a.act = ACT_LEAKY;
        return vsr_launch_conv(dtype, 1, 2, C, C, 0, CO, EPI_NHWC, a, st);
    }
    int point_dgrad(const void* dy, const void* wpackd, void* da, void* db, int N, int H, int W) const {
        ConvArgs a = conv_args(N, H, W, C);
        a.src[0] = dy; a.wpack = wpackd; a.w_zstride = CO * C; a.nz = 2;
        a.dst[0] = da; a.dst[1] = db;
        return vsr_launch_conv(dtype, 1, 1, C, C, 0, CO, EPI_NHWC, a, st);
    }

    int pack_spy(int j, const float* w, void* dst, int mode) const {
        if (mode == 0) return pack(w, dst, 49, SPY_COP[j], SPY_CIP[j], SPY_CO[j], SPY_CI[j], SPY_CI[j], 0, 1, 0, 0);
        return pack(w, dst, 49, SPY_DROWS[j], SPY_DK[j], SPY_CI[j], SPY_CO[j], SPY_CI[j], 0, 1, 0, 1);
    }
    int spy_conv(int j, const void* x, const void* wpack, const float* bias, void* y, int act, float slope, const float* pres, int N, int H, int W) const {
        ConvArgs a = conv_args(N, H, W, SPY_CD[j]);
        a.src[0] = x; a.src_nstride[0] = pm_image_elems(H, W, SPY_CIP[j]);
        a.wpack = wpack; a.bias = bias; a.act = act; a.leaky_slope = slope; a.cout_real = SPY_CO[j]; a.dst[0] = y;
        if (j < NSPY - 1) return vsr_launch_conv(dtype, 7, 1, SPY_CIP[j], SPY_CIP[j], 0, SPY_COP[j], EPI_NHWC, a, st);
        a.dst_nstride = (long long)2 * H * W; a.pres = pres;
        return vsr_launch_conv(dtype, 7, 1, 16, 16, 0, 32, EPI_PLANAR, a, st);
    }
    int spy_dgrad(int j, const void* dy, const void* wpackd, void* dx, const void* aux, int N, int H, int W) const {
        const int CI = SPY_CIP[j], DK = SPY_DK[j];
        ConvArgs a = conv_args(N, H, W, CI);
        a.src[0] = dy; a.src_nstride[0] = pm_image_elems(H, W, DK);
        a.wpack = wpackd; a.dst[0] = dx; a.cout_real = j == 0 ? 8 : CI;
        if (aux) { a.aux[0] = aux; a.mask_mode = MASK_RELU; }
        return vsr_launch_conv(dtype, 7, 1, DK, DK, 0, SPY_DROWS[j], EPI_NHWC, a, st);
    }
    int spy_wgrad(int j, const void* x, const void* dy, int N, int H, int W, float* gw, float* gb, int accumulate) const {
        const int CI = SPY_CIP[j], DK = SPY_DK[j];
        const int nhalf = (dtype == VSR_F32 && CI == 64) ? 2 : 1;
        for (int hf = 0; hf < nhalf; ++hf) {
            WgradArgs a = wg_base(N, H, W, CI, DK);
            a.x[0] = x; a.dy[0] = dy;
            const int cx = CI / nhalf;
            if (nhalf == 2) { a.x_ctotal = CI; a.x_coff = hf * (cx / 8); }
            const int cin_real = nhalf == 2 ? cx : SPY_CI[j];
            CK(wgrad(a, {7, cx, false, DK, false}, {SPY_CO[j], cin_real, gw, SPY_CI[j], hf * cx, 1, 0, hf == 0 ? gb : nullptr, accumulate}));
        }
        return VSR_OK;
    }

    int wgrad(WgradArgs& a, const WgradShape& s, const WgradDst& d, bool even = true) const { return wgrad_run(st, dtype, slab, a, s, d, even); }
    int wgrad_cc(int ks, WgradArgs& a, float* gw, int I_total, int i_off, float* gb, int accumulate) const {
        return wgrad(a, {ks, C, false, C, false}, {C, C, gw, I_total, i_off, 1, 0, gb, accumulate});
    }

    int pack_cc(int ks, const float* w, void* dst, int mode) const { return pack(w, dst, ks * ks, CO, C, C, C, C, 0, 1, 0, mode); }
    int pack(const float* w, void* dst, int KK, int RP, int CPd, int r_real, int c_real, int I_total, int i_off, int o_mul,
             int o_add, int mode) const {
        return pack_any(dtype, w, dst, KK, RP, CPd, r_real, c_real, I_total, i_off, o_mul, o_add, mode);
    }
    int pack_bias(const float* b, void* dst, int nreal, int o_mul = 1, int o_add = 0) const {
        return pack_any(VSR_F32, b, dst, 1, nreal, 1, nreal, 1, 1, 0, o_mul, o_add, 0);
    }
    int pack_any(int dt, const float* w, void* dst, int KK, int RP, int CPd, int r_real, int c_real, int I_total, int i_off, int o_mul,
                 int o_add, int mode) const {
        if (!batch) return vsr_launch_pack_weights(dt, w, dst, KK, RP, CPd, r_real, c_real, I_total, i_off, o_mul, o_add, mode, st);
        VsrPackDesc d = {};
        d.w = w; d.dst = dst; d.total = KK * RP * CPd;
        d.KK = (short)KK; d.RP = (short)RP; d.CPd = (short)CPd; d.r_real = (short)r_real; d.c_real = (short)c_real;
        d.I_total = (short)I_total; d.i_off = (short)i_off; d.o_mul = (short)o_mul; d.o_add = (short)o_add;
        d.mode = (unsigned char)mode; d.dtype = (unsigned char)dt;
        batch->push_back(d);
        return VSR_OK;
    }
};
```

### vsrlab_amd/csrc/wgrad_mfma.hip

```cpp
#include <cstdlib>
#include "elt.h"
#include "kernels.h"

namespace {

constexpr int TW = 32, TH = 8, NTHREADS = 256;

__device__ __forceinline__ void chunk_sum(const uint4& v, float* s) {
    union { uint4 u; bf16_t h[8]; } t; t.u = v;
#pragma unroll
    for (int j = 0; j < 8; ++j) s[j] += (float)t.h[j];
}
__device__ __forceinline__ void chunk_sum(const chunk32_t& v, float* s) {
    s[0] += __uint_as_float(v.a.x); s[1] += __uint_as_float(v.a.y); s[2] += __uint_as_float(v.a.z); s[3] += __uint_as_float(v.a.w);
    s[4] += __uint_as_float(v.b.x); s[5] += __uint_as_float(v.b.y); s[6] += __uint_as_float(v.b.z); s[7] += __uint_as_float(v.b.w);
}

template <int CP> __device__ __forceinline__ int wswz(int pix, int c) {
    return CP == 8 ? (c ^ (((pix >> 1) & 1) << 2)) : c;
}

template <typename T, int CP> __device__ __forceinline__ int lds_addr(int pix, int ch) {
    constexpr int CHB = Elt<T>::CHB;
    return (pix * CP + wswz<CP>(pix, ch >> 3)) * CHB + (ch & 7) * (int)sizeof(T);
}

__device__ uint4 g_wg_zero[4];

template <typename T, int KS, int CX, bool XPLANAR, int COUT, bool DYPLANAR>
__global__ __launch_bounds__(NTHREADS, 2) void wgrad_kernel(const WgradArgs a) {
    constexpr int PAD = KS / 2, KK = KS * KS;
    constexpr int TWH = TW + KS - 1, THH = TH + KS - 1, NPIXX = THH * TWH, NPIXY = TH * TW;
    constexpr int CPX = CX / 8, CPY = COUT / 8;
    constexpr int CHB = Elt<T>::CHB;
    constexpr int NCB = COUT >= 32 ? COUT / 32 : 1;
    constexpr int NIB = CX >= 32 ? CX / 32 : 1;
    constexpr int NT = NCB * NIB;
    constexpr int TAPSPLIT = 4 / NT;
    constexpr int KT = KS == 7 ? 7 : KK;
    constexpr int NTAP = (KT + TAPSPLIT - 1) / TAPSPLIT;
    constexpr int COUTP = NCB * 32, CXP = NIB * 32;
    constexpr int XBYTES = NPIXX * CPX * CHB;
    typedef typename Elt<T>::chunk_t chunk_t;

    extern __shared__ __attribute__((aligned(16))) char smem[];
    char* lx = smem;
    char* ly = smem + XBYTES;

    const int tid = threadIdx.x, lane = tid & 63, wave = tid >> 6;
    const int l31 = lane & 31, h = lane >> 5;
    const int cb = wave % NCB, ib = (wave / NCB) % NIB, tap0 = wave / NT;

    f32x16_t acc[NTAP];
#pragma unroll
    for (int i = 0; i < NTAP; ++i)
#pragma unroll
        for (int j = 0; j < 16; ++j) acc[i][j] = 0.f;
    float bsum[8];
#pragma unroll
    for (int j = 0; j < 8; ++j) bsum[j] = 0.f;

    const int tiles_per_img = a.ntiles_x * a.ntiles_y;
    const int ntiles = a.N * tiles_per_img;

    for (int seg = 0; seg < a.nseg; ++seg) {
        for (int tile = blockIdx.x; tile < ntiles; tile += gridDim.x) {
            const int n = tile / tiles_per_img;
            const int tr = tile - n * tiles_per_img;
            const int ty0 = (tr / a.ntiles_x) * TH, tx0 = (tr % a.ntiles_x) * TW;
            __syncthreads();
            if (XPLANAR) {
                const float* base = reinterpret_cast<const float*>(a.x[seg]) + (long long)n * a.x_nstride;
                const long long plane = (long long)a.Hx * a.Wx;
                const float* zf = reinterpret_cast<const float*>(g_wg_zero);
                for (int p0 = tid; p0 < NPIXX; p0 += 2 * NTHREADS) {
                    float cv[2][3];
#pragma unroll
                    for (int k = 0; k < 2; ++k) {
                        const int p = p0 + k * NTHREADS < NPIXX ? p0 + k * NTHREADS : 0;
                        const int ty = p / TWH, tx = p - ty * TWH;
                        const int vy = ty0 + ty - PAD, vx = tx0 + tx - PAD;
                        const bool in = vy >= 0 && vy < a.H && vx >= 0 && vx < a.W;
                        const float* sp = in ? base + (long long)(vy * a.x_step + a.x_oy) * a.Wx + (vx * a.x_step + a.x_ox) : zf;
                        const long long pl = in ? plane : 0;
                        cv[k][0] = sp[0]; cv[k][1] = sp[pl]; cv[k][2] = sp[2 * pl];
                    }
#pragma unroll
                    for (int k = 0; k < 2; ++k) {
                        const int p = p0 + k * NTHREADS;
                        if (p < NPIXX) {
                            *reinterpret_cast<chunk_t*>(lx + (p * 2 + 0) * CHB) = make_chunk3(cv[k][0], cv[k][1], cv[k][2], (T*)nullptr);
                            *reinterpret_cast<chunk_t*>(lx + (p * 2 + 1) * CHB) = zero_chunk<T>();
                        }
                    }
                }
            } else {
                const T* base = reinterpret_cast<const T*>(a.x[seg]) + (long long)n * a.x_nstride;
                const T* zsrc = reinterpret_cast<const T*>(g_wg_zero);
                for (int idx0 = tid; idx0 < NPIXX * CPX; idx0 += 4 * NTHREADS) {
                    chunk_t v[4];
#pragma unroll
                    for (int k = 0; k < 4; ++k) {
                        const int idx = idx0 + k * NTHREADS, ic = idx < NPIXX * CPX ? idx : 0;
                        const int p = ic / CPX, c = ic - p * CPX;
                        const int ty = p / TWH, tx = p - ty * TWH;
                        const int vy = ty0 + ty - PAD, vx = tx0 + tx - PAD;
                        const bool in = vy >= 0 && vy < a.H && vx >= 0 && vx < a.W;
                        const T* sp = in ? base + pm_off(vy * a.x_step + a.x_oy, vx * a.x_step + a.x_ox, c + a.x_coff, a.Wx, a.x_ctotal ? a.x_ctotal : CX) : zsrc;
                        v[k] = *reinterpret_cast<const chunk_t*>(sp);
                    }
#pragma unroll
                    for (int k = 0; k < 4; ++k) {
                        const int idx = idx0 + k * NTHREADS;
                        if (idx < NPIXX * CPX) {
                            const int p = idx / CPX, c = idx - p * CPX;
                            *reinterpret_cast<chunk_t*>(lx + (p * CPX + wswz<CPX>(p, c)) * CHB) = v[k];
                        }
                    }
                }
            }
            if (DYPLANAR) {
                const float* base = reinterpret_cast<const float*>(a.dy[seg]) + (long long)n * a.dy_nstride;
                const long long plane = (long long)a.Hy * a.Wy;
                const float* zf = reinterpret_cast<const float*>(g_wg_zero);
                for (int p = tid; p < NPIXY; p += NTHREADS) {
                    const int ty = p / TW, tx = p - ty * TW;
                    const int vy = ty0 + ty, vx = tx0 + tx;
                    const int pc = a.dy_planar_c ? a.dy_planar_c : 3;
                    const bool in = vy < a.H && vx < a.W;
                    const float* sp = in ? base + (long long)(vy * a.dy_step + a.dy_oy) * a.Wy + (vx * a.dy_step + a.dy_ox) : zf;
                    const float c0 = sp[0], c1 = *(in && pc > 1 ? sp + plane : zf), c2 = *(in && pc > 2 ? sp + 2 * plane : zf);
                    bsum[0] += c0; bsum[1] += c1; bsum[2] += c2;
                    *reinterpret_cast<chunk_t*>(ly + (p * 2 + 0) * CHB) = make_chunk3(c0, c1, c2, (T*)nullptr);
                    *reinterpret_cast<chunk_t*>(ly + (p * 2 + 1) * CHB) = zero_chunk<T>();
                }
            } else {
                const T* base = reinterpret_cast<const T*>(a.dy[seg]) + (long long)n * a.dy_nstride;
                const T* zsrc = reinterpret_cast<const T*>(g_wg_zero);
                for (int idx0 = tid; idx0 < NPIXY * CPY; idx0 += 4 * NTHREADS) {
                    chunk_t v[4];
#pragma unroll
                    for (int k = 0; k < 4; ++k) {
                        const int idx = idx0 + k * NTHREADS, ic = idx < NPIXY * CPY ? idx : 0;
                        const int p = ic / CPY, c = ic - p * CPY;
                        const int ty = p / TW, tx = p - ty * TW;
                        const int vy = ty0 + ty, vx = tx0 + tx;
                        const bool in = idx < NPIXY * CPY && vy < a.H && vx < a.W;
                        const T* sp = in ? base + pm_off(vy * a.dy_step + a.dy_oy, vx * a.dy_step + a.dy_ox, c + a.dy_coff, a.Wy, a.dy_ctotal ? a.dy_ctotal : COUT) : zsrc;
                        v[k] = *reinterpret_cast<const chunk_t*>(sp);
                    }
#pragma unroll
                    for (int k = 0; k < 4; ++k) {
                        const int idx = idx0 + k * NTHREADS;
                        if (idx < NPIXY * CPY) {
                            const int p = idx / CPY, c = idx - p * CPY;
                            chunk_sum(v[k], bsum);
                            *reinterpret_cast<chunk_t*>(ly + (p * CPY + wswz<CPY>(p, c)) * CHB) = v[k];
                        }
                    }
                }
            }
            __syncthreads();

            for (int row = 0; row < TH; ++row) {
#pragma unroll
                for (int half = 0; half < 2; ++half) {
                    const int xk = half * 16;
                    if constexpr (sizeof(T) == 2) {
                        const int g2 = (lane >> 4) & 1, q = (lane & 15) >> 2, p4 = (lane & 3) * 4;
                        const int chy = cb * 32 + (COUT >= 32 ? 16 * g2 : 0) + p4;
                        const int chx = ib * 32 + (CX >= 32 ? 16 * g2 : 0) + p4;
                        const int py = row * TW + xk + 8 * h + q;
                        const s16x4_t a0 = lds_tr_read(ly + lds_addr<T, CPY>(py, chy));
                        const s16x4_t a1 = lds_tr_read(ly + lds_addr<T, CPY>(py + 4, chy));
                        bf16x8_t af;
                        { union { s16x4_t s[2]; bf16x8_t b; } u; u.s[0] = a0; u.s[1] = a1; af = u.b; }
#pragma unroll
                        for (int i = 0; i < NTAP; ++i) {
                            const int tap = a.tap_begin + tap0 + i * TAPSPLIT;
                            if (tap0 + i * TAPSPLIT < KT) {
                                const int ky = tap / KS, kx = tap - ky * KS;
                                const int px = (row + ky) * TWH + xk + kx + 8 * h + q;
                                const s16x4_t b0 = lds_tr_read(lx + lds_addr<T, CPX>(px, chx));
                                const s16x4_t b1 = lds_tr_read(lx + lds_addr<T, CPX>(px + 4, chx));
                                union { s16x4_t s[2]; bf16x8_t b; } u; u.s[0] = b0; u.s[1] = b1;
                                acc[i] = __builtin_amdgcn_mfma_f32_32x32x16_bf16(af, u.b, acc[i], 0, 0, 0);
                            }
                        }
                    } else {
                        const int chy = cb * 32 + (COUT >= 32 ? l31 : (l31 & 15));
                        const int chx = ib * 32 + (CX >= 32 ? l31 : (l31 & 15));
#pragma unroll
                        for (int j = 0; j < 8; ++j) {
                            const int py = row * TW + xk + 2 * j + h;
                            const float av = *reinterpret_cast<const float*>(ly + lds_addr<T, CPY>(py, chy));
#pragma unroll
                            for (int i = 0; i < NTAP; ++i) {
                                const int tap = a.tap_begin + tap0 + i * TAPSPLIT;
                                if (tap0 + i * TAPSPLIT < KT) {
                                    const int ky = tap / KS, kx = tap - ky * KS;
                                    const int px = (row + ky) * TWH + xk + kx + 2 * j + h;
                                    const float bv = *reinterpret_cast<const float*>(lx + lds_addr<T, CPX>(px, chx));
                                    acc[i] = __builtin_amdgcn_mfma_f32_32x32x2f32(av, bv, acc[i], 0, 0, 0);
                                }
                            }
                        }
                    }
                }
            }
        }
    }

    float* slab = a.slab + (long long)blockIdx.x * a.slab_stride;
#pragma unroll
    for (int i = 0; i < NTAP; ++i) {
        const int tap = a.tap_begin + tap0 + i * TAPSPLIT;
        if (tap0 + i * TAPSPLIT < KT) {
#pragma unroll
            for (int r = 0; r < 16; ++r) {
                const int co = cb * 32 + (r & 3) + 8 * (r >> 2) + 4 * h;
                slab[((long long)tap * COUTP + co) * CXP + ib * 32 + l31] = acc[i][r];
            }
        }
    }
    __syncthreads();
    float* red = reinterpret_cast<float*>(smem);
#pragma unroll
    for (int j = 0; j < 8; ++j) red[tid * 8 + j] = bsum[j];
    __syncthreads();
    if (tid < COUTP) {
        float s = 0.f;
        if (DYPLANAR) {
            if (tid < 3) for (int t = 0; t < NTHREADS; ++t) s += red[t * 8 + tid];
        } else if (tid < COUT) {
            const int c = tid >> 3, j = tid & 7;
            for (int t = c; t < NTHREADS; t += CPY) s += red[t * 8 + j];
        }
        slab[(long long)KK * COUTP * CXP + tid] = s;
    }
}

__global__ void wgrad_reduce_kernel(const float* slab, int nwg, int slab_stride, int KK, int COUTP, int CXP,
                                    int cout_real, int cin_real, float* gw, int I_total, int i_off, int o_mul, int o_add,
                                    float* gb, int accumulate) {
    __shared__ float part[4][64];
    const int total = KK * cout_real * cin_real;
    const int e = threadIdx.x & 63, grp = threadIdx.x >> 6;
    const int idx = blockIdx.x * 64 + e;
    const float* p = nullptr;
    float* d = nullptr;
    if (idx < total) {
        const int ci = idx % cin_real;
        const int co = (idx / cin_real) % cout_real;
        const int tap = idx / (cin_real * cout_real);
        p = slab + ((long long)tap * COUTP + co) * CXP + ci;
        d = gw + ((long long)(co * o_mul + o_add) * I_total + i_off + ci) * KK + tap;
    } else if (gb && idx < total + cout_real) {
        const int co = idx - total;
        p = slab + (long long)KK * COUTP * CXP + co;
        d = gb + co * o_mul + o_add;
    }
    float s = 0.f;
    if (p) {
        int w = grp;
        for (; w + 44 < nwg; w += 48) {
            float v[12];
#pragma unroll
            for (int k = 0; k < 12; ++k) v[k] = p[(long long)(w + 4 * k) * slab_stride];
            s += (v[0] + v[1]) + (v[2] + v[3]);
            s += (v[4] + v[5]) + (v[6] + v[7]);
            s += (v[8] + v[9]) + (v[10] + v[11]);
        }
        for (; w + 12 < nwg; w += 16) {
            const float v0 = p[(long long)w * slab_stride], v1 = p[(long long)(w + 4) * slab_stride];
            const float v2 = p[(long long)(w + 8) * slab_stride], v3 = p[(long long)(w + 12) * slab_stride];
            s += (v0 + v1) + (v2 + v3);
        }
        for (; w < nwg; w += 4) s += p[(long long)w * slab_stride];
    }
    part[grp][e] = s;
    __syncthreads();
    if (grp == 0 && d) {
        s = (part[0][e] + part[1][e]) + (part[2][e] + part[3][e]);
        *d = accumulate ? *d + s : s;
    }
}

__global__ void wgrad_reduce_pairs_kernel(const float* __restrict__ slab, int slab_stride, int ksplit, int nsl, int ncob, int views,
                                          float* __restrict__ gw, int cin_total) {
    __shared__ float part[4][64];
    const int e = threadIdx.x & 63, grp = threadIdx.x >> 6;
    const int idx = blockIdx.x * 64 + e;
    const int pair = blockIdx.y;
    const int sl = pair % nsl, o = (pair / nsl) % ncob, v = pair / (nsl * ncob);
    const int ci = idx & 63, co = (idx >> 6) & 63, tap = idx >> 12;
    float* d = nullptr;
    if (views == 1) {
        d = gw + ((long long)(o * 64 + co) * cin_total + sl * 64 + ci) * 9 + tap;
    } else {
        const int dy = tap / 3 - 1, dx = tap % 3 - 1;
        const int ky = (v >> 1) == 0 ? (dy >= 0 ? 2 * dy + 1 : -1) : (dy <= 0 ? 2 * (dy + 1) : -1);
        const int kx = (v & 1) == 0 ? (dx >= 0 ? 2 * dx + 1 : -1) : (dx <= 0 ? 2 * (dx + 1) : -1);
        if (ky >= 0 && kx >= 0) d = gw + ((long long)(o * 64 + co) * cin_total + sl * 64 + ci) * 16 + ky * 4 + kx;
    }
    float s = 0.f;
    if (d) {
        const float* p = slab + (long long)pair * ksplit * slab_stride + idx;
        for (int w = grp; w < ksplit; w += 4) s += p[(long long)w * slab_stride];
    }
    part[grp][e] = s;
    __syncthreads();
    if (grp == 0 && d) *d += (part[0][e] + part[1][e]) + (part[2][e] + part[3][e]);
}

template <typename T, int KS, int CX, bool XP, int COUT, bool DP>
int launch_wgrad_inst(const WgradArgs& a0, int nwg, hipStream_t st) {
    constexpr int TWH = TW + KS - 1, THH = TH + KS - 1;
    constexpr int CHB = Elt<T>::CHB;
    constexpr int LDS_T = THH * TWH * (CX / 8) * CHB + TH * TW * (COUT / 8) * CHB;
    constexpr int LDS = LDS_T > NTHREADS * 8 * 4 ? LDS_T : NTHREADS * 8 * 4;
    static_assert(LDS <= 160 * 1024, "wgrad tiles do not fit LDS");
    auto kern = wgrad_kernel<T, KS, CX, XP, COUT, DP>;
    static VsrDevOnce once;
    { const int rc = vsr_set_max_dynamic_lds(once, reinterpret_cast<const void*>(kern), LDS); if (rc != VSR_OK) return rc; }
    WgradArgs a = a0;
    a.ntiles_x = cdiv(a.W, TW);
    a.ntiles_y = cdiv(a.H, TH);
    for (int tb = 0; tb < KS * KS; tb += (KS == 7 ? 7 : KS * KS)) {
        a.tap_begin = tb;
        hipLaunchKernelGGL(kern, dim3(nwg), dim3(NTHREADS), LDS, st, a);
        HIP_CHECK_RET(hipGetLastError());
    }
    return VSR_OK;
}

__device__ uint4 g_zero_chunk[2];

constexpr int XS = 36, YS = 35;
constexpr int XROW = 8 * XS * 16, YROW = 8 * YS * 16;
constexpr int DXB = (TH + 2) * XROW;
constexpr int DYB = TH * YROW;
constexpr int DSET = DXB + DYB;
constexpr int DX_SLOTS = (TH + 2) * 8 * XS, DY_SLOTS = TH * 8 * YS;
constexpr int DX_PIECES = DX_SLOTS / 64;
constexpr int DY_PIECES = DY_SLOTS / 64;
constexpr int DNT = 512;
static_assert(DX_SLOTS % 64 == 0 && DY_SLOTS % 64 == 0, "whole DMA pieces");

#ifdef VSR_CLOCK
__device__ unsigned long long g_wclk[256 * 4];
#endif
__global__ __launch_bounds__(DNT, 2) void wgrad3x3_c64_pc_kernel(const WgradArgs a) {
    extern __shared__ __attribute__((aligned(16))) char smem[];
    const int tid = threadIdx.x, lane = tid & 63, wave = tid >> 6;
    const int role = __builtin_amdgcn_readfirstlane(wave >> 2);
    const int w4 = __builtin_amdgcn_readfirstlane(wave & 3);
#ifdef VSR_CLOCK
    unsigned long long clk_t0 = 0, clk_r0 = 0, clk_bar = 0, clk_tiles = 0;
    if (tid == 0) { clk_t0 = __builtin_amdgcn_s_memtime(); clk_r0 = __builtin_amdgcn_s_memrealtime(); }
#endif
    const int tiles_per_img = a.ntiles_x * a.ntiles_y;
    const int per_seg = a.N * tiles_per_img;
    const int total = a.nseg * per_seg;
    TileWalk walk = xcd_tile_walk(total, blockIdx.x, gridDim.x);
    int x_coff = a.x_coff, dy_coff = a.dy_coff, x_oy = a.x_oy, x_ox = a.x_ox;
    int slab_idx = blockIdx.x;
    if (a.pair_ksplit > 0) {
        const int kq = a.pair_ksplit >> 3, xcd = blockIdx.x & 7, j = blockIdx.x >> 3;
        const int pair = j / kq, part = xcd + 8 * (j - pair * kq);
        const int s = pair % a.pair_nsl, o = (pair / a.pair_nsl) % a.pair_ncob, v = pair / (a.pair_nsl * a.pair_ncob);
        x_coff = s * 8; dy_coff = o * 8;
        if (a.pair_views > 1) { x_oy = v >> 1; x_ox = v & 1; }
        walk.first = (int)((long long)total * part / a.pair_ksplit);
        walk.end = (int)((long long)total * (part + 1) / a.pair_ksplit);
        walk.stride = 1;
        slab_idx = pair * a.pair_ksplit + part;
    }
    float* slab = a.slab + (long long)slab_idx * a.slab_stride;

    if (role == 1) {
        const char* zsrc = reinterpret_cast<const char*>(g_zero_chunk);
        const int xcp = (a.x_ctotal ? a.x_ctotal : 64) >> 3, ycp = (a.dy_ctotal ? a.dy_ctotal : 64) >> 3;
        constexpr int NPIECE = (DX_PIECES + DY_PIECES) / 4;
        static_assert((DX_PIECES + DY_PIECES) % 4 == 0, "even split over 4 producer waves");
        int rel[NPIECE];
        unsigned padmask = 0;
#pragma unroll
        for (int i = 0; i < NPIECE; ++i) {
            const int piece = w4 + 4 * i;
            if (piece < DX_PIECES) {
                const int idx = piece * 64 + lane;
                const int row = idx / (8 * XS), rem = idx - row * (8 * XS);
                const int c = rem / XS, tx = rem - c * XS;
                const int dx = (tx - 1) * a.x_step + x_ox;
                rel[i] = (((((row - 1) * a.x_step) * pm_ws(a.Wx) + (dx >> 5)) * xcp + c) * 256 + (dx & 31) * 8) * 2;
                if (tx >= TW + 2) padmask |= 1u << i;
            } else {
                const int idx = (piece - DX_PIECES) * 64 + lane;
                const int row = idx / (8 * YS), rem = idx - row * (8 * YS);
                const int c = rem / YS, tx = rem - c * YS - (c & 1);
                const int dx = (tx < 0 ? 0 : tx) * a.dy_step + a.dy_ox;
                rel[i] = ((((row * a.dy_step) * pm_ws(a.Wy) + (dx >> 5)) * ycp + c) * 256 + (dx & 31) * 8) * 2;
                if (tx < 0 || tx >= TW) padmask |= 1u << i;
            }
        }
        struct { int T, seg, n, ty, tx, sseg, sn, sty, stx; } it;
        {
            int r = walk.first;
            it.T = r; it.seg = r / per_seg; r -= it.seg * per_seg; it.n = r / tiles_per_img; r -= it.n * tiles_per_img;
            it.ty = r / a.ntiles_x; it.tx = r - it.ty * a.ntiles_x;
            r = walk.stride;
            it.sseg = r / per_seg; r -= it.sseg * per_seg; it.sn = r / tiles_per_img; r -= it.sn * tiles_per_img;
            it.sty = r / a.ntiles_x; it.stx = r - it.sty * a.ntiles_x;
        }
        auto advance = [&]() {
            it.T += walk.stride;
            it.tx += it.stx; if (it.tx >= a.ntiles_x) { it.tx -= a.ntiles_x; ++it.ty; }
            it.ty += it.sty; if (it.ty >= a.ntiles_y) { it.ty -= a.ntiles_y; ++it.n; }
            it.n += it.sn; if (it.n >= a.N) { it.n -= a.N; ++it.seg; }
            it.seg += it.sseg;
        };
        int cseg = -1;
        const char *xseg = nullptr, *yseg = nullptr;
        auto issue = [&](int s) {
            if (it.seg != cseg) {
                cseg = it.seg;
                xseg = reinterpret_cast<const char*>(a.x[cseg]);
                yseg = reinterpret_cast<const char*>(a.dy[cseg]);
            }
            const int ty0 = it.ty * TH, tx0 = it.tx * TW;
            const char* xb = xseg + (long long)it.n * a.x_nstride * 2;
            const char* yb = yseg + (long long)it.n * a.dy_nstride * 2;
            const char* xo = xb + pm_off(ty0 * a.x_step + x_oy, tx0 * a.x_step, x_coff, a.Wx, xcp * 8) * 2;
            const char* yo = yb + pm_off(ty0 * a.dy_step + a.dy_oy, tx0 * a.dy_step, dy_coff, a.Wy, ycp * 8) * 2;
            char* lxs = smem + s * DSET;
            const bool interior = ty0 >= 1 && ty0 + TH < a.H && tx0 >= 1 && tx0 + TW < a.W;
#pragma unroll
            for (int i = 0; i < NPIECE; ++i) {
                const int piece = w4 + 4 * i;
                const bool isx = piece < DX_PIECES;
                const char* src = (isx ? xo : yo) + rel[i];
                const bool pad = (padmask >> i) & 1u;
                bool valid = true;
                if (!interior && !pad) {
                    if (isx) {
                        const int idx = piece * 64 + lane;
                        const int row = idx / (8 * XS), tx = (idx - row * (8 * XS)) % XS;
                        const int vy = ty0 + row - 1, vx = tx0 + tx - 1;
                        valid = vy >= 0 && vy < a.H && vx >= 0 && vx < a.W;
                    } else {
                        const int idx = (piece - DX_PIECES) * 64 + lane;
                        const int row = idx / (8 * YS), rem = idx - row * (8 * YS), c = rem / YS, tx = rem - c * YS - (c & 1);
                        valid = ty0 + row < a.H && tx0 + tx < a.W;
                    }
                }
                if (!valid) src = zsrc;
                char* dst = isx ? lxs + piece * 1024 : lxs + DXB + (piece - DX_PIECES) * 1024;
                if (!pad) __builtin_amdgcn_global_load_lds((const __attribute__((address_space(1))) void*)src,
                                                           (__attribute__((address_space(3))) void*)dst, 16, 0, 0);
            }
        };
        float bsum[8];
#pragma unroll
        for (int j = 0; j < 8; ++j) bsum[j] = 0.f;
        const int pt = tid - 256;
        int cur = 0;
        if (it.T < walk.end) issue(0);
        asm volatile("s_waitcnt vmcnt(0)" ::: "memory");
        __syncthreads();
        while (it.T < walk.end) {
            const unsigned lyb = (unsigned)(cur * DSET + DXB + (pt & 7) * (YS * 16) + ((pt >> 3) + (pt & 1)) * 16);
            advance();
            if (it.T < walk.end) issue(cur ^ 1);
            uint4 bq[8];
            asm volatile("ds_read_b128 %0, %8\n\tds_read_b128 %1, %8 offset:%9\n\tds_read_b128 %2, %8 offset:%10\n\tds_read_b128 %3, %8 offset:%11\n\t"
                         "ds_read_b128 %4, %8 offset:%12\n\tds_read_b128 %5, %8 offset:%13\n\tds_read_b128 %6, %8 offset:%14\n\tds_read_b128 %7, %8 offset:%15\n\t"
                         "s_waitcnt lgkmcnt(0)"
                         : "=&v"(bq[0]), "=&v"(bq[1]), "=&v"(bq[2]), "=&v"(bq[3]), "=&v"(bq[4]), "=&v"(bq[5]), "=&v"(bq[6]), "=&v"(bq[7])
                         : "v"(lyb), "i"(YROW), "i"(2 * YROW), "i"(3 * YROW), "i"(4 * YROW), "i"(5 * YROW), "i"(6 * YROW), "i"(7 * YROW) : "memory");
#pragma unroll
            for (int i = 0; i < 8; ++i) chunk_sum(bq[i], bsum);
            asm volatile("s_waitcnt vmcnt(0)" ::: "memory");
            __syncthreads();
            cur ^= 1;
        }
        __syncthreads();
        float* red = reinterpret_cast<float*>(smem);
#pragma unroll
        for (int j = 0; j < 8; ++j) red[pt * 8 + j] = bsum[j];
        __syncthreads();
    } else {
        const int q = lane >> 4, l15 = lane & 15, qq = l15 >> 2, p4 = l15 & 3;
        const int cb = w4 & 1, ib = w4 >> 1;
        const int xoff = (ib * 4 + (p4 >> 1)) * (XS * 16) + (8 * q + qq) * 16 + (p4 & 1) * 8;
        const int yoff = DXB + (cb * 4 + (p4 >> 1)) * (YS * 16) + (8 * q + qq + (p4 >> 1)) * 16 + (p4 & 1) * 8;
        typedef union { s16x4_t s[2]; bf16x8_t b; } frag_u;
        f32x4_t acc[9][2][2];
#pragma unroll
        for (int t = 0; t < 9; ++t)
#pragma unroll
            for (int m = 0; m < 2; ++m)
#pragma unroll
                for (int n = 0; n < 2; ++n) { acc[t][m][n][0] = 0.f; acc[t][m][n][1] = 0.f; acc[t][m][n][2] = 0.f; acc[t][m][n][3] = 0.f; }
        int cur = 0;
        __syncthreads();
        for (int T = walk.first; T < walk.end; T += walk.stride) {
            const unsigned lx = (unsigned)(cur * DSET + xoff);
            const unsigned ly = (unsigned)(cur * DSET + yoff);
            frag_u A[3][2], B[2][6];
#define PC_TRR(dst_, addr_, imm_) asm volatile("ds_read_b64_tr_b16 %0, %1 offset:%2" : "=v"(dst_) : "v"(addr_), "i"(imm_))
#define PC_LDA(r_, mb_, f_) { PC_TRR((f_).s[0], ly, (r_) * YROW + (mb_) * (2 * YS * 16)); PC_TRR((f_).s[1], ly, (r_) * YROW + (mb_) * (2 * YS * 16) + 64); }
#define PC_LDB(R_, fi_, f_) { PC_TRR((f_).s[0], lx, (R_) * XROW + ((fi_) & 1) * (2 * XS * 16) + ((fi_) >> 1) * 16);      \
                              PC_TRR((f_).s[1], lx, (R_) * XROW + ((fi_) & 1) * (2 * XS * 16) + ((fi_) >> 1) * 16 + 64); }
            __builtin_amdgcn_sched_barrier(0);
            PC_LDA(0, 0, A[0][0]) PC_LDA(0, 1, A[0][1])
            PC_LDB(0, 0, B[0][0]) PC_LDB(0, 1, B[0][1]) PC_LDB(0, 2, B[0][2]) PC_LDB(0, 3, B[0][3]) PC_LDB(0, 4, B[0][4]) PC_LDB(0, 5, B[0][5])
            __builtin_amdgcn_sched_barrier(0);
#define PC_PAIR(R_, ky_, fi_, P_, NV_)                                                                                     \
            {                                                                                                              \
                constexpr int r_ = (R_) - (ky_), t_ = (ky_) * 3 + ((fi_) >> 1), nb_ = (fi_) & 1;                           \
                acc[t_][0][nb_] = __builtin_amdgcn_mfma_f32_16x16x32_bf16(A[r_ % 3][0].b, B[(R_) & 1][fi_].b, acc[t_][0][nb_], 0, 0, 0); \
                acc[t_][1][nb_] = __builtin_amdgcn_mfma_f32_16x16x32_bf16(A[r_ % 3][1].b, B[(R_) & 1][fi_].b, acc[t_][1][nb_], 0, 0, 0); \
                __builtin_amdgcn_sched_barrier(0);                                                                         \
                if ((P_) < 6 && (R_) + 1 <= 9) PC_LDB((R_) + 1, P_, B[((R_) + 1) & 1][P_])                                 \
                if ((R_) + 1 <= 7 && (P_) == ((NV_) >= 2 ? 6 : 4)) PC_LDA((R_) + 1, 0, A[((R_) + 1) % 3][0])                \
                if ((R_) + 1 <= 7 && (P_) == ((NV_) >= 2 ? 7 : 5)) PC_LDA((R_) + 1, 1, A[((R_) + 1) % 3][1])                \
                __builtin_amdgcn_sched_barrier(0);                                                                         \
            }
#define PC_GRP(R_, ky_, P0_, NV_) PC_PAIR(R_, ky_, 0, (P0_), NV_) PC_PAIR(R_, ky_, 1, (P0_) + 1, NV_) PC_PAIR(R_, ky_, 2, (P0_) + 2, NV_) \
                                  PC_PAIR(R_, ky_, 3, (P0_) + 3, NV_) PC_PAIR(R_, ky_, 4, (P0_) + 4, NV_) PC_PAIR(R_, ky_, 5, (P0_) + 5, NV_)
#define PC_TOP { asm volatile("s_waitcnt lgkmcnt(0)" ::: "memory"); __builtin_amdgcn_sched_barrier(0); }
            PC_TOP PC_GRP(0, 0, 0, 1)
            PC_TOP PC_GRP(1, 1, 0, 2) PC_GRP(1, 0, 6, 2)
            PC_TOP PC_GRP(2, 2, 0, 3) PC_GRP(2, 1, 6, 3) PC_GRP(2, 0, 12, 3)
            PC_TOP PC_GRP(3, 2, 0, 3) PC_GRP(3, 1, 6, 3) PC_GRP(3, 0, 12, 3)
            PC_TOP PC_GRP(4, 2, 0, 3) PC_GRP(4, 1, 6, 3) PC_GRP(4, 0, 12, 3)
            PC_TOP PC_GRP(5, 2, 0, 3) PC_GRP(5, 1, 6, 3) PC_GRP(5, 0, 12, 3)
            PC_TOP PC_GRP(6, 2, 0, 3) PC_GRP(6, 1, 6, 3) PC_GRP(6, 0, 12, 3)
            PC_TOP PC_GRP(7, 2, 0, 3) PC_GRP(7, 1, 6, 3) PC_GRP(7, 0, 12, 3)
            PC_TOP PC_GRP(8, 2, 0, 2) PC_GRP(8, 1, 6, 2)
            PC_TOP PC_GRP(9, 2, 0, 1)
#undef PC_TOP
#undef PC_GRP
#undef PC_PAIR
#undef PC_LDB
#undef PC_LDA
#undef PC_TRR
#ifdef VSR_CLOCK
            unsigned long long b0; asm volatile("s_waitcnt lgkmcnt(0)\n\ts_memtime %0\n\ts_waitcnt lgkmcnt(0)" : "=s"(b0) :: "memory");
#endif
            __syncthreads();
#ifdef VSR_CLOCK
            unsigned long long b1; asm volatile("s_memtime %0\n\ts_waitcnt lgkmcnt(0)" : "=s"(b1) :: "memory");
            clk_bar += b1 - b0; ++clk_tiles;
#endif
            cur ^= 1;
        }
#pragma unroll
        for (int t = 0; t < 9; ++t)
#pragma unroll
            for (int m = 0; m < 2; ++m)
#pragma unroll
                for (int n = 0; n < 2; ++n)
#pragma unroll
                    for (int j = 0; j < 4; ++j)
                        slab[((long long)t * 64 + cb * 32 + m * 16 + 4 * q + j) * 64 + ib * 32 + n * 16 + l15] = acc[t][m][n][j];
        __syncthreads();
        __syncthreads();
        if (tid < 64) {
            const float* red = reinterpret_cast<const float*>(smem);
            float s = 0.f;
            const int c = tid >> 3, j = tid & 7;
            for (int t = c; t < 256; t += 8) s += red[t * 8 + j];
            slab[9 * 64 * 64 + tid] = s;
        }
    }
#ifdef VSR_CLOCK
    if (tid == 0 && blockIdx.x < 256) {
        g_wclk[blockIdx.x * 4 + 0] = __builtin_amdgcn_s_memtime() - clk_t0;
        g_wclk[blockIdx.x * 4 + 1] = __builtin_amdgcn_s_memrealtime() - clk_r0;
        g_wclk[blockIdx.x * 4 + 2] = clk_bar;
        g_wclk[blockIdx.x * 4 + 3] = clk_tiles;
    }
#endif
}

int launch_wgrad_pc(const WgradArgs& a0, int nwg, hipStream_t st) {
    constexpr int LDS = 2 * DSET;
    static VsrDevOnce once;
    { const int rc = vsr_set_max_dynamic_lds(once, reinterpret_cast<const void*>(wgrad3x3_c64_pc_kernel), LDS); if (rc != VSR_OK) return rc; }
    WgradArgs a = a0;
    a.ntiles_x = cdiv(a.W, TW);
    a.ntiles_y = cdiv(a.H, TH);
    hipLaunchKernelGGL(wgrad3x3_c64_pc_kernel, dim3(nwg), dim3(DNT), LDS, st, a);
    HIP_CHECK_RET(hipGetLastError());
    return VSR_OK;
}

}

#ifdef VSR_CLOCK
extern "C" int vsr_debug_read_wclk(unsigned long long* host_out) {
    return hipMemcpyFromSymbol(host_out, HIP_SYMBOL(g_wclk), sizeof(unsigned long long) * 256 * 4) == hipSuccess ? 0 : -3;
}
#endif



#define VSR_WGRAD_SHAPES(X)           \
    X(3, 64, false, 64, false)         \
    X(3, 16, true, 64, false)          \
    X(3, 64, false, 16, true)          \
    X(1, 64, false, 64, false)         \
    X(7, 16, false, 32, false)         \
    X(7, 32, false, 64, false)         \
    X(7, 64, false, 32, false)         \
    X(7, 32, false, 32, false)        \
    X(7, 32, false, 16, false)         \
    X(7, 16, false, 16, false)         \
     \
    X(3, 16, false, 16, false)         \
    X(3, 32, false, 32, false)         \
    X(3, 16, true, 16, false)          \
    X(3, 16, true, 32, false)          \
    X(1, 16, false, 16, false)         \
    X(1, 32, false, 32, false)        \
    X(3, 16, false, 64, false)         \
    X(3, 32, false, 64, false)        \
    X(3, 16, false, 16, true)          \
    X(3, 32, false, 16, true)

int vsr_launch_wgrad7x7_pc(int cx, int cout, const WgradArgs& a, int max_slabs, int* nslabs, hipStream_t st);

void vsr_wgrad_slab_dims(int ks, int cx, int cout, int* coutp, int* cxp, int* stride) {
    const int ncb = cout >= 32 ? cout / 32 : 1, nib = cx >= 32 ? cx / 32 : 1;
    *coutp = ncb * 32;
    *cxp = nib * 32;
    *stride = ks * ks * (*coutp) * (*cxp) + (*coutp);
}

int vsr_launch_wgrad(int dtype, int ks, int cx, int x_planar, int cout, int dy_planar,
                     const WgradArgs& a, int nwg, int* nslabs, hipStream_t st) {
    if (a.nseg < 1 || a.nseg > VSR_WG_MAXSEG || nwg < 1 || !nslabs) return VSR_ERR_BADARG;
    *nslabs = nwg;
    {
        const bool force_generic = vsr_env().generic_wgrad;
        if (!force_generic && dtype == VSR_BF16 && ks == 3 && cx == 64 && !x_planar && cout == 64 && !dy_planar && nwg >= 2) {
            *nslabs = nwg / 2;
            return launch_wgrad_pc(a, nwg / 2, st);
        }
    }
    if (!vsr_env().generic_wgrad && dtype == VSR_BF16 && ks == 3 && cx == 64 && !x_planar && cout == 16 && dy_planar && a.nseg == 1 && a.x_step == 1 &&
        a.dy_step == 1 && !a.x_oy && !a.x_ox && !a.dy_oy && !a.dy_ox && a.Hx == a.H && a.Wx == a.W && a.Hy == a.H && a.Wy == a.W && !a.x_ctotal && !a.x_coff &&
        a.x_nstride == pm_image_elems(a.H, a.W, 64)) {
        const int rc = vsr_launch_last2_wgrad(a.x[0], reinterpret_cast<const float*>(a.dy[0]), a.dy_nstride, a.slab, a.slab_stride, a.N, a.H, a.W, nslabs, st,
                                              a.dy_planar_c ? a.dy_planar_c : 3);
        if (rc != VSR_ERR_UNSUPPORTED) return rc;
        *nslabs = nwg;
    }
    if (!vsr_env().generic_wgrad && dtype == VSR_BF16 && ks == 7 && !x_planar && !dy_planar) {
        const int rc = vsr_launch_wgrad7x7_pc(cx, cout, a, nwg, nslabs, st);
        if (rc != VSR_ERR_UNSUPPORTED) return rc;
        *nslabs = nwg;
    }
#define X(KS, CX, XP, COUT, DP)                                                                        \
    if (ks == KS && cx == CX && (x_planar != 0) == XP && cout == COUT && (dy_planar != 0) == DP) {    \
        if (dtype == VSR_BF16) return launch_wgrad_inst<bf16_t, KS, CX, XP, COUT, DP>(a, nwg, st);    \
        if (dtype == VSR_F32) {                                                                       \
            if constexpr (KS == 7 && CX == 64) return VSR_ERR_UNSUPPORTED;                             \
            else return launch_wgrad_inst<float, KS, CX, XP, COUT, DP>(a, nwg, st);                   \
        }                                                                                             \
        return VSR_ERR_BADARG;                                                                        \
    }
    VSR_WGRAD_SHAPES(X)
#undef X
    return VSR_ERR_UNSUPPORTED;
}

int vsr_launch_wgrad_reduce(const float* slab, int nwg, int ks, int cx, int cout, int cout_real, int cin_real,
                            float* gw, int I_total, int i_off, int o_mul, int o_add, float* gb, int accumulate,
                            hipStream_t st) {
    int coutp, cxp, stride;
    vsr_wgrad_slab_dims(ks, cx, cout, &coutp, &cxp, &stride);
    const int total = ks * ks * cout_real * cin_real + (gb ? cout_real : 0);
    hipLaunchKernelGGL(wgrad_reduce_kernel, dim3(cdiv(total, 64)), dim3(256), 0, st, slab, nwg, stride, ks * ks,
                       coutp, cxp, cout_real, cin_real, gw, I_total, i_off, o_mul, o_add, gb, accumulate);
    HIP_CHECK_RET(hipGetLastError());
    return VSR_OK;
}

int vsr_launch_wgrad_pairs(int dtype, const WgradArgs& a0, int nsl, int ncob, int views, int ksplit, float* gw, int cin_total, hipStream_t st) {
    if (dtype != VSR_BF16) return VSR_ERR_UNSUPPORTED;
    if (nsl < 1 || ncob < 1 || (views != 1 && views != 4) || ksplit < 8 || (ksplit & 7) || a0.nseg < 1 || a0.nseg > VSR_WG_MAXSEG) return VSR_ERR_BADARG;
    const int npairs = nsl * ncob * views;
    if ((long long)npairs * ksplit > VSR_WGRAD_MAX_PAIR_SLABS) return VSR_ERR_BADARG;
    constexpr int LDS = 2 * DSET;
    static VsrDevOnce once;
    { const int rc = vsr_set_max_dynamic_lds(once, reinterpret_cast<const void*>(wgrad3x3_c64_pc_kernel), LDS); if (rc != VSR_OK) return rc; }
    WgradArgs a = a0;
    a.ntiles_x = cdiv(a.W, TW);
    a.ntiles_y = cdiv(a.H, TH);
    a.pair_ksplit = ksplit; a.pair_nsl = nsl; a.pair_ncob = ncob; a.pair_views = views;
    hipLaunchKernelGGL(wgrad3x3_c64_pc_kernel, dim3(npairs * ksplit), dim3(DNT), LDS, st, a);
    HIP_CHECK_RET(hipGetLastError());
    hipLaunchKernelGGL(wgrad_reduce_pairs_kernel, dim3(9 * 64, npairs), dim3(256), 0, st, a.slab, a.slab_stride, ksplit, nsl, ncob, views, gw, cin_total);
    HIP_CHECK_RET(hipGetLastError());
    return VSR_OK;
}
```

Baseline: 56.37 LR frames/s.

## Batch trunk residual-block weight-gradient convs into multi-job wgrad launches

Instead of launching one wgrad kernel and one reduce per residual-block conv (60 convs for 30 blocks), the trunk wgrad pass now builds a job list and runs a jobs variant of the MFMA wgrad kernel. Each workgroup walks its tiles for several convs in turn and writes per-job partial slabs, and a batched reduce kernel with a y-grid over jobs follows. Groups are capped by slab size (VSR_WG_GROUP=6 jobs), which enlarges the workspace slabs. This is meant to cut launch overhead and tail idle time between many small kernels. The cost is more slab memory and a more complex kernel with per-job flush synchronisations.

```diff
diff --git a/__graft_entry__.py b/__graft_entry__.py
--- a/__graft_entry__.py
+++ b/__graft_entry__.py
@@ -27,6 +27,7 @@
     vsrlab_amd._lib.load_spatial_corr()
     vsrlab_amd._lib.load_jpeg()
     vsrlab_amd._lib.load_warp_taps()
+    vsrlab_amd._lib.load_trunk_jobs_hook()
 
 
 def smoke() -> None:
diff --git a/vsrlab_amd/_lib.py b/vsrlab_amd/_lib.py
--- a/vsrlab_amd/_lib.py
+++ b/vsrlab_amd/_lib.py
@@ -181,7 +181,16 @@
 }
 WARP_TAPS_EXPORTS = tuple(WARP_TAPS_SIGNATURES)
 
+TRUNK_JOBS_HOOK_LIB_PATH = os.path.join(_HERE, "lib", "libvsrlab_trunk_jobs_hook.so")
+TRUNK_JOBS_HOOK_SIGNATURES = {
+    "vsr_debug_trunk_wgrad_jobs": (c_int, [c_int, c_int, _P, _P, c_int, c_int, _P, _P, _P, c_int, c_int, _P, _LL, _P, _P]),
+    "vsr_debug_trunk_wgrad_jobs_slab_floats": (_LL, [c_int]),
+    "vsr_debug_trunk_wgrad_jobs_group": (c_int, [c_int]),
+    "vsr_debug_trunk_wgrad_jobs_cap": (c_int, []),
+}
+
 _lib = None
+_trunk_jobs_hook_lib = None
 _spatial_corr_lib = None
 _jpeg_lib = None
 _warp_taps_lib = None
@@ -201,6 +210,23 @@
             fn.argtypes = args
         _warp_taps_lib = lib
     return _warp_taps_lib
+
+
+def load_trunk_jobs_hook():
+    global _trunk_jobs_hook_lib
+    if _trunk_jobs_hook_lib is None:
+        load()
+        if not os.path.exists(TRUNK_JOBS_HOOK_LIB_PATH):
+            raise RuntimeError(
+                f"vsrlab_amd: HIP library not built ({TRUNK_JOBS_HOOK_LIB_PATH} missing). Run "
+                "`python -c 'import __graft_entry__ as g; g.build()'` or `make -C vsrlab_amd/csrc`.")
+        lib = ctypes.CDLL(TRUNK_JOBS_HOOK_LIB_PATH)
+        for name, (res, args) in TRUNK_JOBS_HOOK_SIGNATURES.items():
+            fn = getattr(lib, name)
+            fn.restype = res
+            fn.argtypes = args
+        _trunk_jobs_hook_lib = lib
+    return _trunk_jobs_hook_lib
 
 
 def load_jpeg():
diff --git a/vsrlab_amd/csrc/common.h b/vsrlab_amd/csrc/common.h
--- a/vsrlab_amd/csrc/common.h
+++ b/vsrlab_amd/csrc/common.h
@@ -78,6 +78,17 @@
     int pair_ksplit, pair_nsl, pair_ncob, pair_views;
 };
 
+#define VSR_WG_MAXJOBS 60
+struct WgradJobArgs {
+    const char* base;
+    float* slab;
+    long long x_nstride, dy_nstride, job_stride;
+    int nseg, N, H, W, njobs, slab_stride, ntiles_x, ntiles_y;
+    unsigned seg[VSR_WG_MAXJOBS][2][VSR_WG_MAXSEG];
+};
+struct WgradReduceJob { float* gw; float* gb; int i_off, o_add; };
+struct WgradReduceJobs { WgradReduceJob job[VSR_WG_MAXJOBS]; };
+
 static inline __host__ __device__ int cdiv(int a, int b) { return (a + b - 1) / b; }
 static inline int grid_for(long long total, int block = 256) {
     long long g = (total + block - 1) / block;
diff --git a/vsrlab_amd/csrc/engine.hip b/vsrlab_amd/csrc/engine.hip
--- a/vsrlab_amd/csrc/engine.hip
+++ b/vsrlab_amd/csrc/engine.hip
@@ -34,6 +34,7 @@
     std::vector<size_t> G0[2], G1[2], DX[2];
     std::vector<size_t> dFeatB, dFF;
     size_t S[2] = {}, dWp[2] = {}, slab[2] = {};
+    int wg_group = 1;
     size_t far_cnt = 0;
     size_t chain_sync[2] = {0, 0};
     bool chains = true;
@@ -150,7 +151,8 @@
                     GU1f[i] = ups == 2 ? b.take(gu1) : GU0f[i];
                     GPf[i] = b.take(a1);
                 }
-            for (int k = 0; k < 2; ++k) slab[k] = b.take(wgrad_slab_bytes());
+            wg_group = diet || dtype != VSR_BF16 || C != 64 ? 1 : (2 * rb < VSR_WG_GROUP ? 2 * rb : VSR_WG_GROUP);
+            for (int k = 0; k < 2; ++k) slab[k] = b.take(wgrad_jobs_slab_floats(wg_group) * 4);
         }
         for (int dir = 0; dir < 2; ++dir) chain_sync[dir] = sb ? b.take(vsr_chain_sync_bytes(VSR_CHAIN_MAX_LAYERS, n, h, w)) : 0;
         dflows = 0;
@@ -167,7 +169,7 @@
 };
 
 Ctx engine_ctx(const Plan& p, char* ws, hipStream_t st, int lane) {
-    return Ctx(ws, st, p.dtype, p.C, p.bwd ? reinterpret_cast<float*>(ws + p.slab[lane]) : nullptr);
+    return Ctx(ws, st, p.dtype, p.C, p.bwd ? reinterpret_cast<float*>(ws + p.slab[lane]) : nullptr, wgrad_jobs_slab_floats(p.wg_group));
 }
 
 struct PIdx {
@@ -544,10 +546,25 @@
     return VSR_OK;
 }
 int trunk_wgrads(const Ctx& c, const Plan& p, int dir, const float* lrs, float* const* g) {
+    const PIdx ix{p.rb, p.ups};
+    std::vector<WgradJob> jobs((size_t)2 * p.rb);
     for (int i0 = 0; i0 < p.t; i0 += VSR_WG_MAXSEG) {
         const int i1 = i0 + VSR_WG_MAXSEG < p.t ? i0 + VSR_WG_MAXSEG : p.t;
         CK(stem_wgrads(c, p, dir, i0, i1, lrs, g));
-        for (int b = 0; b < p.rb; ++b) CK(block_wgrads(c, p, dir, b, i0, i1, g));
+        WgradArgs shape = wg_base(p.n, p.h, p.w, p.C, p.C);
+        shape.nseg = i1 - i0;
+        for (int b = 0; b < p.rb; ++b) {
+            WgradJob& j1 = jobs[2 * b];
+            WgradJob& j2 = jobs[2 * b + 1];
+            j1 = {}; j2 = {};
+            for (int i = i0; i < i1; ++i) {
+                j1.x[i - i0] = c.at(p.xoff(dir, i, b)); j1.dy[i - i0] = c.at(p.g1off(dir, i, b));
+                j2.x[i - i0] = c.at(p.aoff(dir, i, b)); j2.dy[i - i0] = c.at(p.dxoff(dir, i, b + 1));
+            }
+            j1.gw = g[ix.blk_w(dir, 2 * b)]; j1.gb = g[ix.blk_b(dir, 2 * b)];
+            j2.gw = g[ix.blk_w(dir, 2 * b + 1)]; j2.gb = g[ix.blk_b(dir, 2 * b + 1)];
+        }
+        CK(c.wgrad_cc_jobs(shape, jobs.data(), 2 * p.rb, p.C, 0, 1));
     }
     return VSR_OK;
 }
diff --git a/vsrlab_amd/csrc/host.h b/vsrlab_amd/csrc/host.h
--- a/vsrlab_amd/csrc/host.h
+++ b/vsrlab_amd/csrc/host.h
@@ -65,3 +65,76 @@
     return vsr_launch_wgrad_reduce(slab, nslabs, s.ks, s.cx, s.cout, d.cout_real, d.cin_real, d.gw, d.I_total, d.i_off, d.o_mul, d.o_add, d.gb,
                                    d.accumulate, st);
 }
+
+#define VSR_WG_GROUP 6
+struct WgradJob { const void* x[VSR_WG_MAXSEG]; const void* dy[VSR_WG_MAXSEG]; float* gw; float* gb; };
+inline int wgrad_job_slabs(int N, int H, int W) {
+    const long long tiles = (long long)N * cdiv(H, 8) * cdiv(W, 32);
+    const int nwg = (int)(tiles < VSR_WGRAD_NWG ? tiles : VSR_WGRAD_NWG) & ~1;
+    return nwg / 2;
+}
+inline size_t wgrad_jobs_slab_floats(int jobs) {
+    const size_t f = (size_t)jobs * (VSR_WGRAD_NWG / 2) * wgrad_slab_stride3();
+    return f > wgrad_slab_floats() ? f : wgrad_slab_floats();
+}
+inline int wgrad_jobs_run(hipStream_t st, int dtype, int C, float* slab, size_t slab_floats, const WgradArgs& shape, const WgradJob* jobs, int njobs,
+                          int I_total, int i_off, int accumulate, int* nlaunch = nullptr) {
+    if (nlaunch) *nlaunch = 0;
+    if (!jobs || njobs < 1 || !slab || shape.nseg < 1 || shape.nseg > VSR_WG_MAXSEG || bad_dims(shape.N, shape.H, shape.W) ||
+        slab_floats < wgrad_slab_floats() || shape.pair_ksplit > 0)
+        return VSR_ERR_BADARG;
+    if (shape.x_step != 1 || shape.dy_step != 1 || shape.x_oy || shape.x_ox || shape.dy_oy || shape.dy_ox || shape.Hx != shape.H || shape.Wx != shape.W ||
+        shape.Hy != shape.H || shape.Wy != shape.W || shape.x_ctotal || shape.x_coff || shape.dy_ctotal || shape.dy_coff)
+        return VSR_ERR_UNSUPPORTED;
+    for (int k = 0; k < njobs; ++k) {
+        if (!jobs[k].gw) return VSR_ERR_BADARG;
+        for (int s = 0; s < shape.nseg; ++s) if (!jobs[k].x[s] || !jobs[k].dy[s]) return VSR_ERR_BADARG;
+    }
+    const int nslabs = wgrad_job_slabs(shape.N, shape.H, shape.W), stride = wgrad_slab_stride3();
+    bool list = dtype == VSR_BF16 && C == 64 && !vsr_env().generic_wgrad && nslabs >= 1 && njobs > 1;
+    uintptr_t base = ~(uintptr_t)0;
+    if (list) {
+        for (int k = 0; k < njobs; ++k)
+            for (int s = 0; s < shape.nseg; ++s) {
+                const uintptr_t px = (uintptr_t)jobs[k].x[s], py = (uintptr_t)jobs[k].dy[s];
+                base = px < base ? px : base; base = py < base ? py : base;
+            }
+        for (int k = 0; k < njobs && list; ++k)
+            for (int s = 0; s < shape.nseg; ++s) {
+                const uintptr_t dx = (uintptr_t)jobs[k].x[s] - base, dy = (uintptr_t)jobs[k].dy[s] - base;
+                if (((dx | dy) & 255) || ((dx | dy) >> 40)) { list = false; break; }
+            }
+    }
+    if (!list) {
+        for (int k = 0; k < njobs; ++k) {
+            WgradArgs a = shape;
+            for (int s = 0; s < shape.nseg; ++s) { a.x[s] = jobs[k].x[s]; a.dy[s] = jobs[k].dy[s]; }
+            CK(wgrad_run(st, dtype, slab, a, {3, C, false, C, false}, {C, C, jobs[k].gw, I_total, i_off, 1, 0, jobs[k].gb, accumulate}));
+            if (nlaunch) ++*nlaunch;
+        }
+        return VSR_OK;
+    }
+    const long long job_stride = (long long)nslabs * stride;
+    const size_t fit = slab_floats / (size_t)job_stride;
+    const int group = (int)(fit < VSR_WG_MAXJOBS ? fit : VSR_WG_MAXJOBS);
+    for (int k0 = 0; k0 < njobs; k0 += group) {
+        const int nj = k0 + group < njobs ? group : njobs - k0;
+        WgradJobArgs j = {};
+        WgradReduceJob r[VSR_WG_MAXJOBS];
+        j.base = reinterpret_cast<const char*>(base); j.slab = slab; j.job_stride = job_stride; j.slab_stride = stride;
+        j.x_nstride = shape.x_nstride; j.dy_nstride = shape.dy_nstride;
+        j.nseg = shape.nseg; j.N = shape.N; j.H = shape.H; j.W = shape.W; j.njobs = nj;
+        for (int k = 0; k < nj; ++k) {
+            const WgradJob& jb = jobs[k0 + k];
+            for (int s = 0; s < shape.nseg; ++s) {
+                j.seg[k][0][s] = (unsigned)(((uintptr_t)jb.x[s] - base) >> 8);
+                j.seg[k][1][s] = (unsigned)(((uintptr_t)jb.dy[s] - base) >> 8);
+            }
+            r[k] = {jb.gw, jb.gb, i_off, 0};
+        }
+        CK(vsr_launch_wgrad_jobs(j, nslabs, st));
+        if (nlaunch) ++*nlaunch;
+        CK(vsr_launch_wgrad_reduce_jobs(slab, job_stride, nslabs, r, nj, I_total, 1, accumulate, st));
+    }
+    return VSR_OK;
+}
diff --git a/vsrlab_amd/csrc/kernels.h b/vsrlab_amd/csrc/kernels.h
--- a/vsrlab_amd/csrc/kernels.h
+++ b/vsrlab_amd/csrc/kernels.h
@@ -23,6 +23,9 @@
                      int* nslabs, hipStream_t st);
 int vsr_launch_wgrad_reduce(const float* slab, int nwg, int ks, int cx, int cout, int cout_real, int cin_real, float* gw,
                             int I_total, int i_off, int o_mul, int o_add, float* gb, int accumulate, hipStream_t st);
+int vsr_launch_wgrad_jobs(const WgradJobArgs& j, int nwg, hipStream_t st);
+int vsr_launch_wgrad_reduce_jobs(const float* slab, long long job_stride, int nslabs, const WgradReduceJob* jobs, int njobs, int I_total, int o_mul,
+                                 int accumulate, hipStream_t st);
 int vsr_launch_warp_fwd(int dtype, const void* in, const float* flow, void* out, int N, int H, int W, int C,
                         long long flow_nstride, hipStream_t st, int border = 0);
 int vsr_launch_warp_bwd(int dtype, const void* dout, const float* flow, float* dacc, int N, int H, int W, int C,
diff --git a/vsrlab_amd/csrc/recipes.h b/vsrlab_amd/csrc/recipes.h
--- a/vsrlab_amd/csrc/recipes.h
+++ b/vsrlab_amd/csrc/recipes.h
@@ -18,9 +18,11 @@
     int C, CO;
     size_t es;
     float* slab;
+    size_t slab_floats;
     mutable std::vector<VsrPackDesc>* batch = nullptr;
-    Ctx(char* ws_, hipStream_t st_, int dtype_, int C_ = 64, float* slab_ = nullptr)
-        : ws(ws_), st(st_), dtype(dtype_), C(C_), CO(C_ < 32 ? 32 : C_), es(esize(dtype_)), slab(slab_) {}
+    Ctx(char* ws_, hipStream_t st_, int dtype_, int C_ = 64, float* slab_ = nullptr, size_t slab_floats_ = 0)
+        : ws(ws_), st(st_), dtype(dtype_), C(C_), CO(C_ < 32 ? 32 : C_), es(esize(dtype_)), slab(slab_),
+          slab_floats(slab_floats_ ? slab_floats_ : wgrad_slab_floats()) {}
     void* at(size_t off) const { return ws + off; }
     const float* fat(size_t off) const { return reinterpret_cast<const float*>(ws + off); }
 
@@ -178,6 +180,10 @@
         return wgrad(a, {ks, C, false, C, false}, {C, C, gw, I_total, i_off, 1, 0, gb, accumulate});
     }
 
+    int wgrad_cc_jobs(const WgradArgs& shape, const WgradJob* jobs, int njobs, int I_total, int i_off, int accumulate, int* nlaunch = nullptr) const {
+        return wgrad_jobs_run(st, dtype, C, slab, slab_floats, shape, jobs, njobs, I_total, i_off, accumulate, nlaunch);
+    }
+
     int pack_cc(int ks, const float* w, void* dst, int mode) const { return pack(w, dst, ks * ks, CO, C, C, C, C, 0, 1, 0, mode); }
     int pack(const float* w, void* dst, int KK, int RP, int CPd, int r_real, int c_real, int I_total, int i_off, int o_mul,
              int o_add, int mode) const {
diff --git a/vsrlab_amd/csrc/trunk_jobs_hook.hip b/vsrlab_amd/csrc/trunk_jobs_hook.hip
--- /dev/null
+++ b/vsrlab_amd/csrc/trunk_jobs_hook.hip
@@ -0,0 +1,36 @@
+#include "recipes.h"
+
+extern "C" {
+
+int vsr_debug_trunk_wgrad_jobs(int dtype, int C, const void* const* x, const void* const* dy, int nseg, int njobs, const int* nhw, float* const* gw,
+                               float* const* gb, int accumulate, int pair_ksplit, float* slab, long long slab_floats, int* nlaunch, void* stream) {
+    if (nlaunch) *nlaunch = 0;
+    if (bad_dtype(dtype) || (C != 16 && C != 32 && C != 64) || !x || !dy || !nhw || !gw || !slab || (accumulate & ~1) || nseg < 1 ||
+        nseg > VSR_WG_MAXSEG || njobs < 1 || njobs > 4096 || pair_ksplit != 0 || slab_floats < (long long)wgrad_slab_floats())
+        return VSR_ERR_BADARG;
+    const int N = nhw[0], H = nhw[1], W = nhw[2];
+    if (bad_dims(N, H, W)) return VSR_ERR_BADARG;
+    for (int k = 1; k < njobs; ++k)
+        if (nhw[3 * k] != N || nhw[3 * k + 1] != H || nhw[3 * k + 2] != W) return VSR_ERR_BADARG;
+    std::vector<WgradJob> jobs((size_t)njobs);
+    for (int k = 0; k < njobs; ++k) {
+        WgradJob& j = jobs[k];
+        j = {};
+        for (int i = 0; i < nseg; ++i) {
+            j.x[i] = x[(size_t)k * nseg + i]; j.dy[i] = dy[(size_t)k * nseg + i];
+            if (!j.x[i] || !j.dy[i]) return VSR_ERR_BADARG;
+        }
+        j.gw = gw[k]; j.gb = gb ? gb[k] : nullptr;
+        if (!j.gw) return VSR_ERR_BADARG;
+    }
+    const Ctx c(nullptr, (hipStream_t)stream, dtype, C, slab, (size_t)slab_floats);
+    WgradArgs shape = wg_base(N, H, W, C, C);
+    shape.nseg = nseg;
+    return c.wgrad_cc_jobs(shape, jobs.data(), njobs, C, 0, accumulate, nlaunch);
+}
+
+long long vsr_debug_trunk_wgrad_jobs_slab_floats(int group) { return group < 1 ? 0 : (long long)wgrad_jobs_slab_floats(group); }
+int vsr_debug_trunk_wgrad_jobs_group(int res_blocks) { return res_blocks < 1 ? 0 : (2 * res_blocks < VSR_WG_GROUP ? 2 * res_blocks : VSR_WG_GROUP); }
+int vsr_debug_trunk_wgrad_jobs_cap(void) { return VSR_WG_MAXJOBS; }
+
+}
diff --git a/vsrlab_amd/csrc/wgrad_mfma.hip b/vsrlab_amd/csrc/wgrad_mfma.hip
--- a/vsrlab_amd/csrc/wgrad_mfma.hip
+++ b/vsrlab_amd/csrc/wgrad_mfma.hip
@@ -240,9 +240,9 @@
     }
 }
 
-__global__ void wgrad_reduce_kernel(const float* slab, int nwg, int slab_stride, int KK, int COUTP, int CXP,
-                                    int cout_real, int cin_real, float* gw, int I_total, int i_off, int o_mul, int o_add,
-                                    float* gb, int accumulate) {
+__device__ __forceinline__ void wgrad_reduce_body(const float* slab, int nwg, int slab_stride, int KK, int COUTP, int CXP,
+                                                  int cout_real, int cin_real, float* gw, int I_total, int i_off, int o_mul, int o_add,
+                                                  float* gb, int accumulate) {
     __shared__ float part[4][64];
     const int total = KK * cout_real * cin_real;
     const int e = threadIdx.x & 63, grp = threadIdx.x >> 6;
@@ -284,6 +284,17 @@
         s = (part[0][e] + part[1][e]) + (part[2][e] + part[3][e]);
         *d = accumulate ? *d + s : s;
     }
+}
+__global__ void wgrad_reduce_kernel(const float* slab, int nwg, int slab_stride, int KK, int COUTP, int CXP,
+                                    int cout_real, int cin_real, float* gw, int I_total, int i_off, int o_mul, int o_add,
+                                    float* gb, int accumulate) {
+    wgrad_reduce_body(slab, nwg, slab_stride, KK, COUTP, CXP, cout_real, cin_real, gw, I_total, i_off, o_mul, o_add, gb, accumulate);
+}
+__global__ void wgrad_reduce_jobs_kernel(const float* slab, long long job_stride, int nwg, int slab_stride, int KK, int COUTP, int CXP,
+                                         int cout_real, int cin_real, int I_total, int o_mul, int accumulate, const WgradReduceJobs t) {
+    const WgradReduceJob& j = t.job[blockIdx.y];
+    wgrad_reduce_body(slab + blockIdx.y * job_stride, nwg, slab_stride, KK, COUTP, CXP, cout_real, cin_real, j.gw, I_total, j.i_off, o_mul, j.o_add,
+                      j.gb, accumulate);
 }
 
 __global__ void wgrad_reduce_pairs_kernel(const float* __restrict__ slab, int slab_stride, int ksplit, int nsl, int ncob, int views,
@@ -350,7 +361,8 @@
 #ifdef VSR_CLOCK
 __device__ unsigned long long g_wclk[256 * 4];
 #endif
-__global__ __launch_bounds__(DNT, 2) void wgrad3x3_c64_pc_kernel(const WgradArgs a) {
+template <bool JOBS>
+__device__ __forceinline__ void wgrad3x3_c64_pc_body(const WgradArgs& a, const WgradJobArgs* jl) {
     extern __shared__ __attribute__((aligned(16))) char smem[];
     const int tid = threadIdx.x, lane = tid & 63, wave = tid >> 6;
     const int role = __builtin_amdgcn_readfirstlane(wave >> 2);
@@ -365,7 +377,19 @@
     TileWalk walk = xcd_tile_walk(total, blockIdx.x, gridDim.x);
     int x_coff = a.x_coff, dy_coff = a.dy_coff, x_oy = a.x_oy, x_ox = a.x_ox;
     int slab_idx = blockIdx.x;
-    if (a.pair_ksplit > 0) {
+    const int njobs = JOBS ? jl->njobs : 1;
+    const long long job_stride = JOBS ? jl->job_stride : 0;
+    const int ntw = walk.first < walk.end ? (walk.end - walk.first + walk.stride - 1) / walk.stride : 0;
+    if constexpr (JOBS) {
+        if (ntw == 0) {
+            for (int j = 0; j < njobs; ++j) {
+                float* sj = a.slab + j * job_stride + (long long)blockIdx.x * a.slab_stride;
+                for (int i = tid; i < 9 * 64 * 64 + 64; i += DNT) sj[i] = 0.f;
+            }
+            return;
+        }
+    }
+    if (!JOBS && a.pair_ksplit > 0) {
         const int kq = a.pair_ksplit >> 3, xcd = blockIdx.x & 7, j = blockIdx.x >> 3;
         const int pair = j / kq, part = xcd + 8 * (j - pair * kq);
         const int s = pair % a.pair_nsl, o = (pair / a.pair_nsl) % a.pair_ncob, v = pair / (a.pair_nsl * a.pair_ncob);
@@ -404,7 +428,7 @@
                 if (tx < 0 || tx >= TW) padmask |= 1u << i;
             }
         }
-        struct { int T, seg, n, ty, tx, sseg, sn, sty, stx; } it;
+        struct Iter { int T, seg, n, ty, tx, sseg, sn, sty, stx; } it;
         {
             int r = walk.first;
             it.T = r; it.seg = r / per_seg; r -= it.seg * per_seg; it.n = r / tiles_per_img; r -= it.n * tiles_per_img;
@@ -420,13 +444,20 @@
             it.n += it.sn; if (it.n >= a.N) { it.n -= a.N; ++it.seg; }
             it.seg += it.sseg;
         };
+        const Iter it0 = it;
+        int ijob = 0;
         int cseg = -1;
         const char *xseg = nullptr, *yseg = nullptr;
         auto issue = [&](int s) {
             if (it.seg != cseg) {
                 cseg = it.seg;
-                xseg = reinterpret_cast<const char*>(a.x[cseg]);
-                yseg = reinterpret_cast<const char*>(a.dy[cseg]);
+                if constexpr (JOBS) {
+                    xseg = jl->base + ((unsigned long long)jl->seg[ijob][0][cseg] << 8);
+                    yseg = jl->base + ((unsigned long long)jl->seg[ijob][1][cseg] << 8);
+                } else {
+                    xseg = reinterpret_cast<const char*>(a.x[cseg]);
+                    yseg = reinterpret_cast<const char*>(a.dy[cseg]);
+                }
             }
             const int ty0 = it.ty * TH, tx0 = it.tx * TW;
             const char* xb = xseg + (long long)it.n * a.x_nstride * 2;
@@ -468,10 +499,9 @@
         if (it.T < walk.end) issue(0);
         asm volatile("s_waitcnt vmcnt(0)" ::: "memory");
         __syncthreads();
-        while (it.T < walk.end) {
+        auto tile = [&](bool more) {
             const unsigned lyb = (unsigned)(cur * DSET + DXB + (pt & 7) * (YS * 16) + ((pt >> 3) + (pt & 1)) * 16);
-            advance();
-            if (it.T < walk.end) issue(cur ^ 1);
+            if (more) issue(cur ^ 1);
             uint4 bq[8];
             asm volatile("ds_read_b128 %0, %8\n\tds_read_b128 %1, %8 offset:%9\n\tds_read_b128 %2, %8 offset:%10\n\tds_read_b128 %3, %8 offset:%11\n\t"
                          "ds_read_b128 %4, %8 offset:%12\n\tds_read_b128 %5, %8 offset:%13\n\tds_read_b128 %6, %8 offset:%14\n\tds_read_b128 %7, %8 offset:%15\n\t"
@@ -482,13 +512,40 @@
             for (int i = 0; i < 8; ++i) chunk_sum(bq[i], bsum);
             asm volatile("s_waitcnt vmcnt(0)" ::: "memory");
             __syncthreads();
-            cur ^= 1;
-        }
-        __syncthreads();
-        float* red = reinterpret_cast<float*>(smem);
-#pragma unroll
-        for (int j = 0; j < 8; ++j) red[pt * 8 + j] = bsum[j];
-        __syncthreads();
+        };
+        if constexpr (JOBS) {
+            int tc = 0, jc = 0;
+            for (int k = njobs * ntw; k > 0; --k) {
+                advance();
+                if (it.T >= walk.end) { it = it0; cseg = -1; ++ijob; }
+                tile(ijob < njobs);
+                if (++tc == ntw) {
+                    float* red = reinterpret_cast<float*>(smem + cur * DSET);
+#pragma unroll
+                    for (int j = 0; j < 8; ++j) { const int f = pt * 8 + j; red[(f >> 8) * 1024 + (f & 255)] = bsum[j]; bsum[j] = 0.f; }
+                    __syncthreads();
+                    if (w4 == 0) {
+                        float s = 0.f;
+                        const int c = pt >> 3, j = pt & 7;
+                        for (int t = c; t < 256; t += 8) { const int f = t * 8 + j; s += red[(f >> 8) * 1024 + (f & 255)]; }
+                        (a.slab + jc * job_stride + (long long)blockIdx.x * a.slab_stride)[9 * 64 * 64 + pt] = s;
+                    }
+                    tc = 0; ++jc;
+                }
+                cur ^= 1;
+            }
+        } else {
+            while (it.T < walk.end) {
+                advance();
+                tile(it.T < walk.end);
+                cur ^= 1;
+            }
+            __syncthreads();
+            float* red = reinterpret_cast<float*>(smem);
+#pragma unroll
+            for (int j = 0; j < 8; ++j) red[pt * 8 + j] = bsum[j];
+            __syncthreads();
+        }
     } else {
         const int q = lane >> 4, l15 = lane & 15, qq = l15 >> 2, p4 = l15 & 3;
         const int cb = w4 & 1, ib = w4 >> 1;
@@ -504,7 +561,21 @@
                 for (int n = 0; n < 2; ++n) { acc[t][m][n][0] = 0.f; acc[t][m][n][1] = 0.f; acc[t][m][n][2] = 0.f; acc[t][m][n][3] = 0.f; }
         int cur = 0;
         __syncthreads();
-        for (int T = walk.first; T < walk.end; T += walk.stride) {
+        auto store_acc = [&](float* sl) {
+            sl += ((long long)cb * 32 + 4 * q) * 64 + ib * 32 + l15;
+            if constexpr (JOBS) asm volatile("" : "+v"(sl));
+#pragma unroll
+            for (int t = 0; t < 9; ++t)
+#pragma unroll
+                for (int m = 0; m < 2; ++m)
+#pragma unroll
+                    for (int n = 0; n < 2; ++n)
+#pragma unroll
+                        for (int j = 0; j < 4; ++j)
+                            sl[(t * 64 + m * 16 + j) * 64 + n * 16] = acc[t][m][n][j];
+        };
+        int tc = 0, jc = 0;
+        for (int T = walk.first, k = njobs * ntw; JOBS ? k > 0 : T < walk.end; T += walk.stride, --k) {
             const unsigned lx = (unsigned)(cur * DSET + xoff);
             const unsigned ly = (unsigned)(cur * DSET + yoff);
             frag_u A[3][2], B[2][6];
@@ -554,25 +625,32 @@
             unsigned long long b1; asm volatile("s_memtime %0\n\ts_waitcnt lgkmcnt(0)" : "=s"(b1) :: "memory");
             clk_bar += b1 - b0; ++clk_tiles;
 #endif
+            if constexpr (JOBS) {
+                if (++tc == ntw) {
+                    __syncthreads();
+                    store_acc(slab + jc * job_stride);
+#pragma unroll
+                    for (int t = 0; t < 9; ++t)
+#pragma unroll
+                        for (int m = 0; m < 2; ++m)
+#pragma unroll
+                            for (int n = 0; n < 2; ++n) { acc[t][m][n][0] = 0.f; acc[t][m][n][1] = 0.f; acc[t][m][n][2] = 0.f; acc[t][m][n][3] = 0.f; }
+                    tc = 0; ++jc;
+                }
+            }
             cur ^= 1;
         }
-#pragma unroll
-        for (int t = 0; t < 9; ++t)
-#pragma unroll
-            for (int m = 0; m < 2; ++m)
-#pragma unroll
-                for (int n = 0; n < 2; ++n)
-#pragma unroll
-                    for (int j = 0; j < 4; ++j)
-                        slab[((long long)t * 64 + cb * 32 + m * 16 + 4 * q + j) * 64 + ib * 32 + n * 16 + l15] = acc[t][m][n][j];
-        __syncthreads();
-        __syncthreads();
-        if (tid < 64) {
-            const float* red = reinterpret_cast<const float*>(smem);
-            float s = 0.f;
-            const int c = tid >> 3, j = tid & 7;
-            for (int t = c; t < 256; t += 8) s += red[t * 8 + j];
-            slab[9 * 64 * 64 + tid] = s;
+        if constexpr (!JOBS) {
+            store_acc(slab);
+            __syncthreads();
+            __syncthreads();
+            if (tid < 64) {
+                const float* red = reinterpret_cast<const float*>(smem);
+                float s = 0.f;
+                const int c = tid >> 3, j = tid & 7;
+                for (int t = c; t < 256; t += 8) s += red[t * 8 + j];
+                slab[9 * 64 * 64 + tid] = s;
+            }
         }
     }
 #ifdef VSR_CLOCK
@@ -583,6 +661,15 @@
         g_wclk[blockIdx.x * 4 + 3] = clk_tiles;
     }
 #endif
+}
+
+__global__ __launch_bounds__(DNT, 2) void wgrad3x3_c64_pc_kernel(const WgradArgs a) { wgrad3x3_c64_pc_body<false>(a, nullptr); }
+__global__ __launch_bounds__(DNT, 2) void wgrad3x3_c64_pc_jobs_kernel(const WgradJobArgs j) {
+    WgradArgs a = {};
+    a.x_nstride = j.x_nstride; a.dy_nstride = j.dy_nstride; a.nseg = j.nseg; a.N = j.N; a.H = j.H; a.W = j.W;
+    a.x_step = 1; a.Hx = j.H; a.Wx = j.W; a.dy_step = 1; a.Hy = j.H; a.Wy = j.W;
+    a.slab = j.slab; a.slab_stride = j.slab_stride; a.ntiles_x = j.ntiles_x; a.ntiles_y = j.ntiles_y;
+    wgrad3x3_c64_pc_body<true>(a, &j);
 }
 
 int launch_wgrad_pc(const WgradArgs& a0, int nwg, hipStream_t st) {
@@ -689,6 +776,39 @@
     return VSR_OK;
 }
 
+int vsr_launch_wgrad_jobs(const WgradJobArgs& j0, int nwg, hipStream_t st) {
+    if (j0.njobs < 1 || j0.njobs > VSR_WG_MAXJOBS || j0.nseg < 1 || j0.nseg > VSR_WG_MAXSEG || nwg < 1 || j0.N < 1 || j0.H < 1 || j0.W < 1 ||
+        !j0.base || !j0.slab || j0.slab_stride < 9 * 64 * 64 + 64 || j0.job_stride < (long long)nwg * j0.slab_stride)
+        return VSR_ERR_BADARG;
+    constexpr int LDS = 2 * DSET;
+    static VsrDevOnce once;
+    { const int rc = vsr_set_max_dynamic_lds(once, reinterpret_cast<const void*>(wgrad3x3_c64_pc_jobs_kernel), LDS); if (rc != VSR_OK) return rc; }
+    WgradJobArgs j = j0;
+    j.ntiles_x = cdiv(j.W, TW);
+    j.ntiles_y = cdiv(j.H, TH);
+    hipLaunchKernelGGL(wgrad3x3_c64_pc_jobs_kernel, dim3(nwg), dim3(DNT), LDS, st, j);
+    HIP_CHECK_RET(hipGetLastError());
+    return VSR_OK;
+}
+int vsr_launch_wgrad_reduce_jobs(const float* slab, long long job_stride, int nslabs, const WgradReduceJob* jobs, int njobs, int I_total, int o_mul,
+                                 int accumulate, hipStream_t st) {
+    if (!slab || !jobs || njobs < 1 || njobs > VSR_WG_MAXJOBS || nslabs < 1) return VSR_ERR_BADARG;
+    int coutp, cxp, stride;
+    vsr_wgrad_slab_dims(3, 64, 64, &coutp, &cxp, &stride);
+    WgradReduceJobs t = {};
+    bool bias = false;
+    for (int k = 0; k < njobs; ++k) {
+        if (!jobs[k].gw) return VSR_ERR_BADARG;
+        t.job[k] = jobs[k];
+        bias = bias || jobs[k].gb;
+    }
+    const int total = 9 * 64 * 64 + (bias ? 64 : 0);
+    hipLaunchKernelGGL(wgrad_reduce_jobs_kernel, dim3(cdiv(total, 64), njobs), dim3(256), 0, st, slab, job_stride, nslabs, stride, 9, coutp, cxp, 64, 64,
+                       I_total, o_mul, accumulate, t);
+    HIP_CHECK_RET(hipGetLastError());
+    return VSR_OK;
+}
+
 int vsr_launch_wgrad_pairs(int dtype, const WgradArgs& a0, int nsl, int ncob, int views, int ksplit, float* gw, int cin_total, hipStream_t st) {
     if (dtype != VSR_BF16) return VSR_ERR_UNSUPPORTED;
     if (nsl < 1 || ncob < 1 || (views != 1 && views != 4) || ksplit < 8 || (ksplit & 7) || a0.nseg < 1 || a0.nseg > VSR_WG_MAXSEG) return VSR_ERR_BADARG;
```

New measurement: 56.33 LR frames/s. No clear change (-0.1%).
